# BioinformaticsToolsmith/MeShClust

Measured on AMD Instinct MI355X. Metric: sequences clustered/sec (+ NW cell-updates/sec) at 1/2/4/8 MI355X, higher is better.
Workload: dtype u8

## Files before the change

include/meshclust_amd.h:

```cpp
#ifndef MESHCLUST_AMD_H
#define MESHCLUST_AMD_H

#include <stddef.h>
#include <stdint.h>

#ifdef __cplusplus
extern "C" {
#endif

#define MC_ABI_VERSION 1

#define MC_OK 0
#define MC_ERR_ARG 1
#define MC_ERR_HIP 2
#define MC_ERR_STATE 3
#define MC_ERR_OOM 4
#define MC_ERR_INPUT 5
#define MC_ERR_UNSUPPORTED 6
#define MC_ERR_TIMEOUT 7

#define MC_FEAT_ALIGN (1 << 0)
#define MC_FEAT_LD (1 << 1)
#define MC_FEAT_MANHATTAN (1 << 2)
#define MC_FEAT_INTERSECTION (1 << 4)
// ... 46 lines not shown
                   const uint64_t *exc_pos, const uint8_t *exc_val, uint64_t nexc, const int32_t *seg,
                   const uint64_t *seg_off);

int mc_kmer_max(mc_ctx *ctx, int k, uint64_t *largest);

int mc_kmer_build(mc_ctx *ctx, int k, int width_bytes);

int mc_get_histograms(mc_ctx *ctx, void *hist, uint64_t *mags);

int mc_distance_keys(mc_ctx *ctx, const uint32_t *pivots, uint32_t npiv, const uint32_t *ids,
                     uint64_t m, uint16_t *keys);

int mc_split_begin(mc_ctx *ctx, const uint32_t *pivots, uint32_t npiv, const uint32_t *order, uint64_t n);
int mc_split_begin_words(mc_ctx *ctx, const uint64_t *words, uint32_t narr, uint64_t n, int depth);
int mc_split_select(mc_ctx *ctx, uint64_t nq, const uint32_t *arr, const uint64_t *pos, uint32_t *ids);
int mc_split_select_words(mc_ctx *ctx, uint64_t nq, const uint32_t *arr, const uint64_t *pos, uint64_t *words);
int mc_split_end(mc_ctx *ctx);

int mc_pair_features(mc_ctx *ctx, const uint32_t *a, const uint32_t *b, uint64_t m,
                     const uint16_t *flags, int nflag, double *raw);

int mc_set_classifier(mc_ctx *ctx, const mc_classifier *cls);

int mc_classify_pairs(mc_ctx *ctx, const uint32_t *a, const uint32_t *b, uint64_t m,
                      uint8_t *similar, double *combo0, double *sum);

#define MC_ASSIGN_NONE 0xffffffffu
int mc_assign(mc_ctx *ctx, const uint32_t *centre_ids, uint32_t C, const uint32_t *query_ids, uint64_t M,
              double sim, uint32_t *best, double *best_val, uint32_t *n_similar, uint64_t *stats);

int mc_revcomp_rows(mc_ctx *ctx, const uint32_t *ids, uint64_t m, void *rows );

#define MC_STRAND_PLUS 1
#define MC_STRAND_MINUS 2
int mc_assign_strands(mc_ctx *ctx, const uint32_t *centre_ids, uint32_t C, const uint32_t *query_ids, uint64_t M,
                      double sim, int strands , uint32_t *best, double *best_val,
                      uint8_t *strand , uint32_t *n_similar, uint64_t *stats);

int mc_kmer_max_strands(mc_ctx *ctx, int k, int strands , uint64_t *largest);
int mc_kmer_build_strands(mc_ctx *ctx, int k, int width_bytes, int strands );
int mc_orient_pairs(mc_ctx *ctx, const uint32_t *a, const uint32_t *b, uint64_t m, uint8_t *strand ,
                    uint64_t *sad );

#define MC_ASSIGN_MAX_TOP 8
int mc_assign_top(mc_ctx *ctx, const uint32_t *centre_ids, uint32_t C, const uint32_t *query_ids, uint64_t M,
                  double sim, int strands , uint32_t K ,
                  uint32_t *hit , double *hit_val , uint8_t *hit_strand ,
                  uint32_t *n_similar , uint64_t *stats );

int mc_nw_identity(mc_ctx *ctx, const uint32_t *a, const uint32_t *b, uint64_t m, double *ident,
                   int32_t *len, int32_t *ids);

int mc_nw_identity_raw(mc_ctx *ctx, const uint8_t *a, const uint64_t *a_off, const uint8_t *b,
                       const uint64_t *b_off, uint64_t m, double *ident, int32_t *len,
                       int32_t *ids, int32_t *score);

int mc_revcomp_sequences(mc_ctx *ctx, const uint32_t *ids, uint64_t m, uint8_t *bytes, uint64_t *off);

#define MC_IDENT_BATCH_PAIRS (1ull << 20)
#define MC_IDENT_BATCH_BYTES (256ull << 20)
int mc_nw_identity_strands(mc_ctx *ctx, const uint32_t *a, const uint32_t *b, const uint8_t *a_minus, uint64_t m,
                           double *ident, int32_t *len, int32_t *ids);

#define MC_QGRAM_NA 0xffffffffu
int mc_qgram_common(mc_ctx *ctx, const uint32_t *a, const uint32_t *b, const uint8_t *a_minus, uint64_t m, int q,
                    uint32_t *common);

#define MC_CIGAR_I 1u
#define MC_CIGAR_D 2u
#define MC_CIGAR_EQ 7u
#define MC_CIGAR_X 8u
#define MC_ALIGN_BATCH_PAIRS (1ull << 16)
#define MC_ALIGN_SCRATCH_BYTES (1ull << 30)
int mc_nw_align_strands(mc_ctx *ctx, const uint32_t *a, const uint32_t *b, const uint8_t *a_minus, uint64_t m,
                        uint32_t *cigar, uint64_t cap, uint64_t *cig_off ,
                        int32_t *score, int32_t *len, int32_t *ids);
int mc_nw_align_profile(mc_ctx *ctx, double *out , int reset);

int mc_set_align_band(mc_ctx *ctx, int mode );
int mc_nw_band_plan(mc_ctx *ctx, const uint32_t *a, const uint32_t *b, const uint8_t *a_minus, uint64_t m,
                    int32_t *w , int32_t *score );
int mc_nw_band_profile(mc_ctx *ctx, double *out , int reset);

#define MC_PILEUP_CH 8
int mc_nw_pileup_strands(mc_ctx *ctx, const uint32_t *a, const uint32_t *b, const uint8_t *a_minus, uint64_t m,
                         const uint32_t *targets, uint32_t nt, uint64_t *row_off ,
                         uint32_t *table , uint64_t cap_rows,
                         int32_t *score, int32_t *len, int32_t *ids );
int mc_nw_pileup_profile(mc_ctx *ctx, double *out , int reset);

#define MC_QUAL_MAX 93
int mc_load_qualities(mc_ctx *ctx, const uint8_t *qual, uint64_t bytes);
int mc_nw_qpileup_strands(mc_ctx *ctx, const uint32_t *a, const uint32_t *b, const uint8_t *a_minus, uint64_t m,
                          const uint32_t *targets, uint32_t nt, uint64_t *row_off ,
                          uint32_t *table, uint32_t *wtable , uint64_t cap_rows,
                          int32_t *score, int32_t *len, int32_t *ids );

#define MC_MSA_GAP '-'
#define MC_MSA_BATCH_BYTES (256ull << 20)
int mc_nw_msa_begin(mc_ctx *ctx, const uint32_t *a, const uint32_t *b, const uint8_t *a_minus, uint64_t m,
                    const uint32_t *targets, uint32_t nt, uint64_t *row_off ,
                    uint32_t *width , uint64_t *block_width ,
                    int32_t *score, int32_t *len, int32_t *ids );
int mc_nw_msa_rows(mc_ctx *ctx, uint64_t first, uint64_t count, uint8_t *out, uint64_t cap, uint64_t *off );
int mc_nw_msa_end(mc_ctx *ctx);
int mc_nw_msa_profile(mc_ctx *ctx, double *out , int reset);

#define MC_MSA_CH 8
int mc_nw_msa_counts(mc_ctx *ctx, uint32_t first_target, uint32_t ntargets, uint64_t *col_off ,
                     uint32_t *counts, uint32_t *wcounts , uint64_t cap_cols);
int mc_nw_msa_counts_profile(mc_ctx *ctx, double *out , int reset);

int mc_nw_msa_sites(mc_ctx *ctx, const uint64_t *site_off , const uint32_t *sites ,
                    uint64_t first, uint64_t count, uint8_t *alleles, uint8_t *quals , uint64_t cap,
                    uint64_t *off );
int mc_nw_msa_sites_profile(mc_ctx *ctx, double *out , int reset);

#define MC_CROSS_RES 8
#define MC_CROSS_MAX_READ (1u << 18)
#define MC_CROSS_BATCH_CANDS (1ull << 20)
int mc_nw_msa_crossover(mc_ctx *ctx, const uint64_t *x, const uint64_t *y, uint64_t nc, int32_t *out );
int mc_nw_msa_crossover_profile(mc_ctx *ctx, double *out , int reset);

int mc_set_order(mc_ctx *ctx, const uint32_t *order, uint64_t n);
int mc_kill(mc_ctx *ctx, uint64_t pos);
int mc_cluster_begin(mc_ctx *ctx, uint32_t first_id);
int mc_scan(mc_ctx *ctx, uint32_t centre_id, uint64_t S, uint64_t E, uint32_t *flagged_pos,
            uint64_t cap, mc_scan_result *res);

#define MC_SHARD_BLOCK 256
int mc_scan_part(mc_ctx *ctx, uint32_t centre_id, uint64_t S, uint64_t E, uint32_t part, uint32_t nparts,
                 uint32_t *flagged_pos, uint64_t cap, mc_scan_result *res);
int mc_scan_commit(mc_ctx *ctx, const uint32_t *flagged_pos, uint64_t n, mc_scan_result *res);

int mc_align_part(mc_ctx *ctx, uint32_t centre_id, uint64_t S, uint64_t E, uint32_t part, uint32_t nparts,
                  double *ident, uint64_t cap, uint64_t *n_part, uint64_t *pairs, uint64_t *cells);
int mc_scan_ident(mc_ctx *ctx, uint32_t centre_id, uint64_t S, uint64_t E, const double *ident,
                  uint32_t *flagged_pos, uint64_t cap, mc_scan_result *res);

int mc_accumulate(mc_ctx *ctx, const uint32_t *bin_lo, const uint64_t *bounds, uint32_t nbins, double sim,
                  uint32_t *centre_ids, uint64_t *member_off, uint32_t *member_ids, uint64_t *nclusters,
                  uint64_t *stats);

uint64_t mc_mailbox_bytes(int world, uint64_t n);
int mc_set_mailbox(mc_ctx *ctx, void *host, uint64_t bytes, int rank, int world, int share);
int mc_ctx_pci_bus_id(mc_ctx *ctx, char *buf, int len);
int mc_accum_plan_info(mc_ctx *ctx, uint32_t nbins, uint32_t info[4]);
int mc_set_accum_grid(mc_ctx *ctx, uint32_t grid);
int mc_accum_reserve(mc_ctx *ctx, uint32_t nbins);
int mc_ctx_partition(mc_ctx *ctx, int slot, int share);

int mc_mean_shift(mc_ctx *ctx, const uint32_t *centre_ids, uint32_t C, const uint64_t *member_off,
                  const uint32_t *members, int delta, uint32_t *new_centre);

int mc_update_iteration(mc_ctx *ctx, const uint32_t *centre_ids, uint32_t C, const uint64_t *member_off,
                        const uint32_t *members, int delta, uint32_t *new_centre, uint8_t *similar,
                        double *combo0, uint64_t *npairs);

int mc_mean_shift_range(mc_ctx *ctx, const uint32_t *centre_ids, uint32_t C, const uint64_t *member_off,
                        const uint32_t *members, int delta, uint32_t j0, uint32_t j1, uint32_t *new_centre);


int mc_classify_values(mc_ctx *ctx, const double *raw, uint64_t m, uint8_t *similar, double *combo0,
                       double *sum);

int mc_mean_shift_select(mc_ctx *ctx, const uint32_t *centre_ids, uint32_t C, const uint64_t *member_off,
// ... 19 lines not shown
```

meshclust_amd/__init__.py:

```python
import ctypes as C
import os
import subprocess

import numpy as np

HERE = os.path.dirname(os.path.abspath(__file__))
ROOT = os.path.dirname(HERE)
LIB_DIR = os.path.join(HERE, "lib")
BIN = os.path.join(HERE, "bin", "meshclust")
GPU_LIB = os.environ.get("MC_GPU_LIB", os.path.join(LIB_DIR, "libmcgpu.so"))
HOST_LIB = os.path.join(LIB_DIR, "libmeshclust.so")
HEADER = os.path.join(ROOT, "include", "meshclust_amd.h")

FEAT_ALIGN, FEAT_LD, FEAT_MANHATTAN = 1, 2, 4
FEAT_INTERSECTION, FEAT_PEARSON, FEAT_KULCZYNSKI2 = 16, 32, 1024
COMBO_SQUARED, COMBO_SELF = 1, 2
ASSIGN_NONE = 0xFFFFFFFF
MC_STRAND_PLUS, MC_STRAND_MINUS = 1, 2
ASSIGN_MAX_TOP = 8
ERR_ARG, ERR_UNSUPPORTED = 1, 6
ERR_STATE = 3
CIGAR_I, CIGAR_D, CIGAR_EQ, CIGAR_X = 1, 2, 7, 8
PILEUP_CH = 8
MSA_GAP = ord("-")
MSA_CH = 8
CROSS_RES = 8
QUAL_MAX = 93
QGRAM_NA = 0xFFFFFFFF
FAMILIES = ("kmer", "keys", "pairs", "scan", "finalize", "mean_shift", "nw", "layout")


class MCError(RuntimeError):
    pass


def build(jobs=8):
    subprocess.run(["make", "-s", "-j%d" % jobs, "-C", os.path.join(HERE, "csrc")], check=True)


class Classifier(C.Structure):
    _fields_ = [
        ("n_single", C.c_int32),
        ("lookup", C.c_uint16 * 8),
        ("is_sim", C.c_int32 * 8),
        ("mins", C.c_double * 8),
        ("maxs", C.c_double * 8),
        ("n_combo", C.c_int32),
        ("combo_kind", C.c_int32 * 8),
        ("combo_len", C.c_int32 * 8),
        ("combo_idx", (C.c_int32 * 4) * 8),
        ("weights", C.c_double * 9),
    ]


class ScanResult(C.Structure):
    _fields_ = [
        ("is_min", C.c_int32),
        ("has_best", C.c_int32),
        ("best_pos", C.c_uint64),
        ("best_val", C.c_double),
        ("n_flagged", C.c_uint64),
        ("new_centre", C.c_uint32),
        ("n_members", C.c_uint32),
        ("nw_pairs", C.c_uint64),
        ("nw_cells", C.c_uint64),
    ]


_gpu = None
_host = None


def _p(a):
    return a.ctypes.data_as(C.c_void_p) if a is not None else None


def gpu_lib():
    global _gpu
    if _gpu is None:
        if not os.path.exists(GPU_LIB):
            raise ImportError("libmcgpu.so not built (run meshclust_amd.build()); no CPU fallback exists")
        lib = C.CDLL(GPU_LIB)
        lib.mc_last_error.restype = C.c_char_p
        lib.mc_ctx_create.argtypes = [C.c_int, C.POINTER(C.c_void_p)]
        lib.mc_ctx_destroy.argtypes = [C.c_void_p]
        for name in ("mc_load_sequences", "mc_load_packed", "mc_kmer_max", "mc_kmer_build", "mc_get_histograms", "mc_distance_keys",
                     "mc_pair_features", "mc_set_classifier", "mc_classify_pairs", "mc_nw_identity",
                     "mc_nw_identity_raw", "mc_set_order", "mc_kill", "mc_cluster_begin", "mc_scan",
                     "mc_mean_shift", "mc_update_iteration", "mc_timers", "mc_classify_values", "mc_mean_shift_select", "mc_accumulate",
                     "mc_scan_part", "mc_scan_commit", "mc_comm_unique_id", "mc_comm_create", "mc_comm_allgather",
                     "mc_comm_stats", "mc_comm_destroy", "mc_sync", "mc_assign", "mc_assign_strands",
                     "mc_revcomp_rows", "mc_assign_top", "mc_revcomp_sequences", "mc_nw_identity_strands",
                     "mc_nw_align_strands", "mc_nw_align_profile", "mc_nw_pileup_strands", "mc_nw_pileup_profile",
                     "mc_kmer_max_strands", "mc_kmer_build_strands", "mc_orient_pairs", "mc_qgram_common"):
            getattr(lib, name).restype = C.c_int
        lib.mc_comm_create.argtypes = [C.c_int, C.c_int, C.c_int, C.c_char_p, C.POINTER(C.c_void_p)]
        lib.mc_comm_allgather.argtypes = [C.c_void_p, C.c_void_p, C.c_uint64, C.c_void_p]
        lib.mc_comm_stats.argtypes = [C.c_void_p, C.POINTER(C.c_uint64), C.POINTER(C.c_uint64)]
        lib.mc_comm_destroy.argtypes = [C.c_void_p, C.c_int]
        lib.mc_assign.argtypes = [C.c_void_p, C.c_void_p, C.c_uint32, C.c_void_p, C.c_uint64, C.c_double,
                                  C.c_void_p, C.c_void_p, C.c_void_p, C.c_void_p]
        lib.mc_assign_strands.argtypes = [C.c_void_p, C.c_void_p, C.c_uint32, C.c_void_p, C.c_uint64, C.c_double, C.c_int,
                                          C.c_void_p, C.c_void_p, C.c_void_p, C.c_void_p, C.c_void_p]
        lib.mc_revcomp_rows.argtypes = [C.c_void_p, C.c_void_p, C.c_uint64, C.c_void_p]
        lib.mc_assign_top.argtypes = [C.c_void_p, C.c_void_p, C.c_uint32, C.c_void_p, C.c_uint64, C.c_double, C.c_int,
                                      C.c_uint32, C.c_void_p, C.c_void_p, C.c_void_p, C.c_void_p, C.c_void_p]
        lib.mc_revcomp_sequences.argtypes = [C.c_void_p, C.c_void_p, C.c_uint64, C.c_void_p, C.c_void_p]
        lib.mc_nw_identity_strands.argtypes = [C.c_void_p, C.c_void_p, C.c_void_p, C.c_void_p, C.c_uint64, C.c_void_p,
                                               C.c_void_p, C.c_void_p]
        lib.mc_qgram_common.argtypes = [C.c_void_p, C.c_void_p, C.c_void_p, C.c_void_p, C.c_uint64, C.c_int, C.c_void_p]
        lib.mc_nw_align_strands.argtypes = [C.c_void_p, C.c_void_p, C.c_void_p, C.c_void_p, C.c_uint64, C.c_void_p,
                                            C.c_uint64, C.c_void_p, C.c_void_p, C.c_void_p, C.c_void_p]
        lib.mc_nw_align_profile.argtypes = [C.c_void_p, C.c_void_p, C.c_int]
        lib.mc_nw_pileup_strands.argtypes = [C.c_void_p, C.c_void_p, C.c_void_p, C.c_void_p, C.c_uint64, C.c_void_p, C.c_uint32,
                                             C.c_void_p, C.c_void_p, C.c_uint64, C.c_void_p, C.c_void_p, C.c_void_p]
        lib.mc_nw_pileup_profile.argtypes = [C.c_void_p, C.c_void_p, C.c_int]
        lib.mc_kmer_max_strands.argtypes = [C.c_void_p, C.c_int, C.c_int, C.POINTER(C.c_uint64)]
        lib.mc_kmer_build_strands.argtypes = [C.c_void_p, C.c_int, C.c_int, C.c_int]
        lib.mc_orient_pairs.argtypes = [C.c_void_p, C.c_void_p, C.c_void_p, C.c_uint64, C.c_void_p, C.c_void_p]
        lib.mc_load_qualities.restype = C.c_int
        lib.mc_load_qualities.argtypes = [C.c_void_p, C.c_void_p, C.c_uint64]
        lib.mc_nw_qpileup_strands.restype = C.c_int
        lib.mc_nw_qpileup_strands.argtypes = [C.c_void_p, C.c_void_p, C.c_void_p, C.c_void_p, C.c_uint64, C.c_void_p, C.c_uint32,
                                              C.c_void_p, C.c_void_p, C.c_void_p, C.c_uint64, C.c_void_p, C.c_void_p, C.c_void_p]
        for name in ("mc_nw_msa_begin", "mc_nw_msa_rows", "mc_nw_msa_end", "mc_nw_msa_profile"):
            getattr(lib, name).restype = C.c_int
        lib.mc_nw_msa_begin.argtypes = [C.c_void_p, C.c_void_p, C.c_void_p, C.c_void_p, C.c_uint64, C.c_void_p, C.c_uint32,
                                        C.c_void_p, C.c_void_p, C.c_void_p, C.c_void_p, C.c_void_p, C.c_void_p]
        lib.mc_nw_msa_rows.argtypes = [C.c_void_p, C.c_uint64, C.c_uint64, C.c_void_p, C.c_uint64, C.c_void_p]
        lib.mc_nw_msa_end.argtypes = [C.c_void_p]
        lib.mc_nw_msa_profile.argtypes = [C.c_void_p, C.c_void_p, C.c_int]
        lib.mc_nw_msa_counts.restype = C.c_int
        lib.mc_nw_msa_counts.argtypes = [C.c_void_p, C.c_uint32, C.c_uint32, C.c_void_p, C.c_void_p, C.c_void_p, C.c_uint64]
        lib.mc_nw_msa_counts_profile.restype = C.c_int
        lib.mc_nw_msa_counts_profile.argtypes = [C.c_void_p, C.c_void_p, C.c_int]
        lib.mc_nw_msa_sites.restype = C.c_int
        lib.mc_nw_msa_sites.argtypes = [C.c_void_p, C.c_void_p, C.c_void_p, C.c_uint64, C.c_uint64, C.c_void_p, C.c_void_p, C.c_uint64,
                                        C.c_void_p]
        lib.mc_nw_msa_sites_profile.restype = C.c_int
        lib.mc_nw_msa_sites_profile.argtypes = [C.c_void_p, C.c_void_p, C.c_int]
        lib.mc_nw_msa_crossover.restype = C.c_int
        lib.mc_nw_msa_crossover.argtypes = [C.c_void_p, C.c_void_p, C.c_void_p, C.c_uint64, C.c_void_p]
        lib.mc_nw_msa_crossover_profile.restype = C.c_int
        lib.mc_nw_msa_crossover_profile.argtypes = [C.c_void_p, C.c_void_p, C.c_int]
        for name in ("mc_set_align_band", "mc_nw_band_plan", "mc_nw_band_profile"):
            getattr(lib, name).restype = C.c_int
        lib.mc_set_align_band.argtypes = [C.c_void_p, C.c_int]
        lib.mc_nw_band_plan.argtypes = [C.c_void_p, C.c_void_p, C.c_void_p, C.c_void_p, C.c_uint64, C.c_void_p, C.c_void_p]
        lib.mc_nw_band_profile.argtypes = [C.c_void_p, C.c_void_p, C.c_int]
        _bind_steps(lib)
        _gpu = lib
    return _gpu


def _bind_steps(lib):
    vp, u32, u64 = C.c_void_p, C.c_uint32, C.c_uint64
    lib.mc_set_order.argtypes = [vp, vp, u64]
    lib.mc_kill.argtypes = [vp, u64]
    lib.mc_cluster_begin.argtypes = [vp, u32]
    lib.mc_scan.argtypes = [vp, u32, u64, u64, vp, u64, C.POINTER(ScanResult)]
    lib.mc_scan_part.argtypes = [vp, u32, u64, u64, u32, u32, vp, u64, C.POINTER(ScanResult)]
    lib.mc_scan_commit.argtypes = [vp, vp, u64, C.POINTER(ScanResult)]
    lib.mc_align_part.argtypes = [vp, u32, u64, u64, u32, u32, vp, u64, C.POINTER(u64), C.POINTER(u64), C.POINTER(u64)]
    lib.mc_scan_ident.argtypes = [vp, u32, u64, u64, vp, vp, u64, C.POINTER(ScanResult)]
    lib.mc_mean_shift_range.argtypes = [vp, vp, u32, vp, vp, C.c_int, u32, u32, vp]
    for name in ("mc_set_order", "mc_kill", "mc_cluster_begin", "mc_scan", "mc_scan_part", "mc_scan_commit",
                 "mc_align_part", "mc_scan_ident", "mc_mean_shift_range", "mc_mean_shift"):
        getattr(lib, name).restype = C.c_int
    lib.mc_last_error.restype = C.c_char_p


def load_engine_lib(path):
    lib = C.CDLL(path)
    lib.mc_ctx_create.argtypes = [C.c_int, C.POINTER(C.c_void_p)]
    lib.mc_ctx_destroy.argtypes = [C.c_void_p]
    _bind_steps(lib)
    return lib


def host_lib():
    global _host
    if _host is None:
        if not os.path.exists(HOST_LIB):
            raise ImportError("libmeshclust.so not built (run meshclust_amd.build())")
        gpu_lib()
        lib = C.CDLL(HOST_LIB)
        lib.mcl_parse.restype = C.c_void_p
        lib.mcl_parse.argtypes = [C.POINTER(C.c_char_p), C.c_int, C.c_int, C.c_char_p, C.c_int]
        lib.mcl_parse_q.restype = C.c_void_p
        lib.mcl_parse_q.argtypes = lib.mcl_parse.argtypes
        lib.mcl_qualities.restype = None
        lib.mcl_qualities.argtypes = [C.c_void_p, C.POINTER(C.c_void_p), C.POINTER(C.c_uint64)]
        lib.mcl_num_seqs.restype = C.c_uint64
# ... 299 lines not shown
        r = ScanResult()
        rc = self.lib.mc_scan_part(self.ctx, int(centre), int(S), int(E), int(part), int(nparts), _p(fl), cap, C.byref(r))
        return rc, _scan_dict(r), fl[:min(int(r.n_flagged), cap)].copy() if rc == 0 else fl[:0]

    def scan_commit(self, flagged):
        fl = np.ascontiguousarray(flagged, np.uint32)
        r = ScanResult()
        rc = self.lib.mc_scan_commit(self.ctx, _p(fl) if len(fl) else None, len(fl), C.byref(r))
        return rc, _scan_dict(r)

    def align_part(self, centre, S, E, part, nparts, cap=None):
        cap = max(int(E) - int(S) + 1, 1) if cap is None else int(cap)
        ident = np.zeros(max(cap, 1))
        n, pairs, cells = C.c_uint64(0), C.c_uint64(0), C.c_uint64(0)
        rc = self.lib.mc_align_part(self.ctx, int(centre), int(S), int(E), int(part), int(nparts), _p(ident), cap,
                                    C.byref(n), C.byref(pairs), C.byref(cells))
        return rc, ident[:min(n.value, cap)].copy() if rc == 0 else ident[:0], pairs.value, cells.value

    def scan_ident(self, centre, S, E, ident, cap=None):
        cap = max(int(E) - int(S) + 1, 1) if cap is None else int(cap)
        ident = np.ascontiguousarray(ident, np.float64)
        fl = np.zeros(max(cap, 1), np.uint32)
        r = ScanResult()
        rc = self.lib.mc_scan_ident(self.ctx, int(centre), int(S), int(E), _p(ident), _p(fl), cap, C.byref(r))
        return rc, _scan_dict(r), fl[:min(int(r.n_flagged), cap)].copy() if rc == 0 else fl[:0]

    def mean_shift_range(self, centres, member_off, members, delta, j0, j1):
        centres = np.ascontiguousarray(centres, np.uint32)
        member_off = np.ascontiguousarray(member_off, np.uint64)
        members = np.ascontiguousarray(members, np.uint32)
        out = np.zeros(max(int(j1) - int(j0), 1), np.uint32)
        rc = self.lib.mc_mean_shift_range(self.ctx, _p(centres), len(centres), _p(member_off), _p(members), int(delta),
                                          int(j0), int(j1), _p(out))
        return rc, out[:max(int(j1) - int(j0), 0)]

    def mean_shift_select(self, centres, member_off, members, delta, keep):
        centres = np.ascontiguousarray(centres, np.uint32)
        member_off = np.ascontiguousarray(member_off, np.uint64)
        members = np.ascontiguousarray(members, np.uint32)
        keep = np.ascontiguousarray(keep, np.uint8)
        out = np.zeros(len(centres), np.uint32)
        self._ck(self.lib.mc_mean_shift_select(self.ctx, _p(centres), len(centres), _p(member_off), _p(members), delta,
                                             _p(keep), _p(out)), "mc_mean_shift_select")
        return out

    def nw_identity(self, a, b):
        a = np.ascontiguousarray(a, np.uint32)
        b = np.ascontiguousarray(b, np.uint32)
        ident = np.zeros(len(a))
        ln = np.zeros(len(a), np.int32)
        ids = np.zeros(len(a), np.int32)
        self._ck(self.lib.mc_nw_identity(self.ctx, _p(a), _p(b), C.c_uint64(len(a)), _p(ident), _p(ln), _p(ids)),
               "mc_nw_identity")
        return ident, ln, ids

    def revcomp_sequences(self, ids):
        ids = np.ascontiguousarray(ids, np.uint32)
        off = np.zeros(len(ids) + 1, np.uint64)
        self._ck(self.lib.mc_revcomp_sequences(self.ctx, _p(ids), len(ids), None, _p(off)), "mc_revcomp_sequences")
        out = np.zeros(int(off[-1]), np.uint8)
        self._ck(self.lib.mc_revcomp_sequences(self.ctx, _p(ids), len(ids), _p(out), _p(off)), "mc_revcomp_sequences")
        return out, off

    def nw_identity_strands(self, a, b, a_minus=None):
        a = np.ascontiguousarray(a, np.uint32)
        b = np.ascontiguousarray(b, np.uint32)
        am = None if a_minus is None else np.ascontiguousarray(a_minus, np.uint8)
        assert am is None or len(am) == len(a)
        ident = np.zeros(len(a))
        ln = np.zeros(len(a), np.int32)
        ids = np.zeros(len(a), np.int32)
        self._ck(self.lib.mc_nw_identity_strands(self.ctx, _p(a), _p(b), _p(am), C.c_uint64(len(a)), _p(ident), _p(ln),
                                               _p(ids)), "mc_nw_identity_strands")
        return ident, ln, ids

    def qgram_common(self, a, b, q, a_minus=None):
        a = np.ascontiguousarray(a, np.uint32)
        b = np.ascontiguousarray(b, np.uint32)
        am = None if a_minus is None else np.ascontiguousarray(a_minus, np.uint8)
        assert len(a) == len(b) and (am is None or len(am) == len(a))
        out = np.zeros(len(a), np.uint32)
        self._ck(self.lib.mc_qgram_common(self.ctx, _p(a), _p(b), _p(am), C.c_uint64(len(a)), int(q), _p(out)), "mc_qgram_common")
        return out

    def nw_align_strands(self, a, b, a_minus=None, cigar=True):
        a = np.ascontiguousarray(a, np.uint32)
        b = np.ascontiguousarray(b, np.uint32)
        am = None if a_minus is None else np.ascontiguousarray(a_minus, np.uint8)
        assert len(b) == len(a) and (am is None or len(am) == len(a))
        m = len(a)
        off = np.zeros(m + 1, np.uint64)
        sc = np.zeros(m, np.int32)
        ln = np.zeros(m, np.int32)
        ids = np.zeros(m, np.int32)
        if not cigar:
            self._ck(self.lib.mc_nw_align_strands(self.ctx, _p(a), _p(b), _p(am), C.c_uint64(m), None, C.c_uint64(0), _p(off),
                                                _p(sc), _p(ln), _p(ids)), "mc_nw_align_strands")
            return None, off, sc, ln, ids
        cap = 0
        for x in (a, b):
            self._ck(self.lib.mc_revcomp_sequences(self.ctx, _p(x), m, None, _p(off)), "mc_revcomp_sequences")
            cap += int(off[-1])
        words = np.zeros(cap, np.uint32)
        self._ck(self.lib.mc_nw_align_strands(self.ctx, _p(a), _p(b), _p(am), C.c_uint64(m), _p(words), C.c_uint64(cap), _p(off),
                                            _p(sc), _p(ln), _p(ids)), "mc_nw_align_strands")
        return words[:int(off[-1])], off, sc, ln, ids

    def nw_align_profile(self, reset=False):
        out = np.zeros(3)
        self._ck(self.lib.mc_nw_align_profile(self.ctx, _p(out), 1 if reset else 0), "mc_nw_align_profile")
        return float(out[0]), float(out[1]), float(out[2])

    def set_align_band(self, mode):
        self._ck(self.lib.mc_set_align_band(self.ctx, int(mode)), "mc_set_align_band")

    def nw_band_plan(self, a, b, a_minus=None):
        a = np.ascontiguousarray(a, np.uint32)
        b = np.ascontiguousarray(b, np.uint32)
        am = None if a_minus is None else np.ascontiguousarray(a_minus, np.uint8)
        assert len(b) == len(a) and (am is None or len(am) == len(a))
        w = np.zeros(len(a), np.int32)
        sc = np.zeros(len(a), np.int32)
        self._ck(self.lib.mc_nw_band_plan(self.ctx, _p(a), _p(b), _p(am), C.c_uint64(len(a)), _p(w), _p(sc)), "mc_nw_band_plan")
        return w, sc

    def nw_band_profile(self, reset=False):
        out = np.zeros(5)
        self._ck(self.lib.mc_nw_band_profile(self.ctx, _p(out), 1 if reset else 0), "mc_nw_band_profile")
        return int(out[0]), int(out[1]), int(out[2]), float(out[3]), int(out[4])

    def nw_pileup_strands(self, a, b, a_minus, targets, table=True):
        a = np.ascontiguousarray(a, np.uint32)
        b = np.ascontiguousarray(b, np.uint32)
        am = None if a_minus is None else np.ascontiguousarray(a_minus, np.uint8)
        tg = np.ascontiguousarray(targets, np.uint32)
        assert len(b) == len(a) and (am is None or len(am) == len(a))
        m, nt = len(a), len(tg)
        off = np.zeros(nt + 1, np.uint64)
        sc = np.zeros(m, np.int32)
        ln = np.zeros(m, np.int32)
        ids = np.zeros(m, np.int32)
        self._ck(self.lib.mc_nw_pileup_strands(self.ctx, _p(a), _p(b), _p(am), C.c_uint64(m), _p(tg), C.c_uint32(nt), _p(off), None,
                                             C.c_uint64(0), None, None, None), "mc_nw_pileup_strands")
        if not table:
            return None, off, sc, ln, ids
        rows = int(off[-1])
        tab = np.zeros((rows, PILEUP_CH), np.uint32)
        self._ck(self.lib.mc_nw_pileup_strands(self.ctx, _p(a), _p(b), _p(am), C.c_uint64(m), _p(tg), C.c_uint32(nt), _p(off),
                                             _p(tab), C.c_uint64(rows), _p(sc), _p(ln), _p(ids)), "mc_nw_pileup_strands")
        return tab, off, sc, ln, ids

    def load_qualities(self, q):
        q = np.ascontiguousarray(q, np.uint8)
        self._ck(self.lib.mc_load_qualities(self.ctx, _p(q), C.c_uint64(len(q))), "mc_load_qualities")

    def nw_qpileup_strands(self, a, b, a_minus, targets):
        a = np.ascontiguousarray(a, np.uint32)
        b = np.ascontiguousarray(b, np.uint32)
        am = None if a_minus is None else np.ascontiguousarray(a_minus, np.uint8)
        tg = np.ascontiguousarray(targets, np.uint32)
        assert len(b) == len(a) and (am is None or len(am) == len(a))
        m, nt = len(a), len(tg)
        off = np.zeros(nt + 1, np.uint64)
        sc = np.zeros(m, np.int32)
        ln = np.zeros(m, np.int32)
        ids = np.zeros(m, np.int32)
# ... 297 lines not shown
```

meshclust_amd/csrc/gpu/abi.hip:

```cpp
#include <hip/hip_runtime.h>

#include <algorithm>
#include <chrono>
#include <cfloat>
#include <cmath>
#include <cstdio>
#include <cstdlib>
#include <cstring>
#include <map>
#include <mutex>
#include <string>
#include <thread>
#include <vector>

#include "abi_util.hpp"
#include "mcgpu.hpp"

namespace mcg {

static thread_local std::string g_err;

void set_error(const std::string &m) { g_err = m; }

int hip_fail(hipError_t e, const char *what) {
// ... 147 lines not shown
  MCG_CHECK(hipStreamSynchronize(s));
  if (pinned) {
    size_t off = 0;
    for (const DPart &p : parts)
      if (p.h && p.bytes) {
        memcpy(p.h, c->h_dstage + off, p.bytes);
        off += (p.bytes + 255) / 256 * 256;
      }
  }
  return MC_OK;
}

int download_pinned(mc_ctx *c, const void *d, size_t bytes, hipStream_t s, uint8_t **h) {
  *h = nullptr;
  if (bytes > c->h_dstage_cap) {
    if (c->h_dstage) (void)hipHostFree(c->h_dstage);
    c->h_dstage = nullptr;
    c->h_dstage_cap = 0;
    const size_t cap = std::max<size_t>(bytes, 1u << 20);
    if (hipHostMalloc((void **)&c->h_dstage, cap, hipHostMallocDefault) != hipSuccess) {
      (void)hipGetLastError();
      c->h_dstage = nullptr;
      return MC_OK;
    }
    c->h_dstage_cap = cap;
  }
  if (d) {
    MCG_CHECK(hipMemcpyAsync(c->h_dstage, d, bytes, hipMemcpyDeviceToHost, s));
    MCG_CHECK(hipStreamSynchronize(s));
  }
  *h = c->h_dstage;
  return MC_OK;
}

}

using namespace mcg;

extern "C" {

const char *mc_last_error(void) { return mcg::g_err.c_str(); }
int mc_abi_version(void) { return MC_ABI_VERSION; }

int mc_ctx_create(int device, mc_ctx **out) {
  if (!out) return MC_ERR_ARG;
  int ndev = 0;
  hipError_t e = hipGetDeviceCount(&ndev);
  if (e != hipSuccess || ndev == 0) {
    set_error("no HIP device available (libmcgpu requires an MI355X / gfx950 GPU)");
    return MC_ERR_HIP;
  }
  if (device < 0 || device >= ndev) {
    set_error("device index out of range");
    return MC_ERR_ARG;
  }
  MCG_CHECK(hipSetDevice(device));
  hipDeviceProp_t prop;
  MCG_CHECK(hipGetDeviceProperties(&prop, device));
  if (std::string(prop.gcnArchName).find("gfx950") == std::string::npos) {
    set_error(std::string("libmcgpu is built for gfx950, device is ") + prop.gcnArchName);
    return MC_ERR_HIP;
  }
  auto *c = new mc_ctx();
  c->device = device;
  MCG_CHECK(hipStreamCreateWithFlags(&c->stream, hipStreamNonBlocking));
  MCG_CHECK(hipEventCreate(&c->ev0));
  MCG_CHECK(hipEventCreate(&c->ev1));
  c->cls.thr = decision_threshold();
  *out = c;
  return MC_OK;
}

static void mailbox_detach(mc_ctx *c);

int mc_ctx_destroy(mc_ctx *c) {
  if (!c) return MC_OK;
  (void)hipSetDevice(c->device);
  (void)hipStreamSynchronize(c->stream);
  mailbox_detach(c);
  for (Buf *b : {&c->codes, &c->seq_off, &c->seg, &c->seg_off, &c->packed, &c->pk_off, &c->impure, &c->hist, &c->mag, &c->sumsq, &c->len, &c->order,
                 &c->alive, &c->members, &c->member_keys, &c->partials, &c->scan_dev, &c->flags_out, &c->s_a, &c->s_b,
                 &c->s_c, &c->s_d, &c->s_e, &c->s_f, &c->s_g, &c->s_h, &c->s_i, &c->s_j, &c->s_k, &c->hs, &c->mag_s, &c->sumsq_s, &c->len_s, &c->ticket,
                 &c->msum, &c->ident_s, &c->al_a, &c->al_b, &c->al_out, &c->al_id, &c->ord_ids, &c->acc_out, &c->sp_words, &c->sp_keys,
                 &c->sp_scr, &c->sp_nodes, &c->sp_nn, &c->sp_q, &c->sp_err, &c->u_off, &c->u_mem, &c->nw_items, &c->nw_gran, &c->rc_seq, &c->tr_choice, &c->tr_bnd, &c->tr_ops, &c->tr_pairs, &c->tr_res, &c->tr_idx, &c->tr_dst,
                 &c->tr_out, &c->tr_err, &c->bs_pairs, &c->bs_bnd, &c->bs_score, &c->pu_table, &c->pu_diff, &c->pu_rows, &c->pu_toff, &c->pu_roff, &c->qual, &c->pu_wtable, &c->pu_qoff, &c->msa_width, &c->msa_col, &c->msa_words, &c->msa_bw, &c->msa_rec, &c->msa_out, &c->msa_cnt, &c->msa_wcnt, &c->msa_cdiff, &c->msa_crec, &c->msa_ctgt, &c->msa_scol, &c->msa_sres, &c->msa_stgt, &c->msa_srec, &c->msa_sout, &c->msa_sq, &c->msa_xrec, &c->msa_xout, &c->hist_fwd, &c->or_runs})
    release(*b);
  if (c->h_scan) (void)hipHostFree(c->h_scan);
  if (c->h_stage) (void)hipHostFree(c->h_stage);
  if (c->h_dstage) (void)hipHostFree(c->h_dstage);
  if (c->h_res) (void)hipHostFree(c->h_res);
  for (auto e : c->ev_pool) (void)hipEventDestroy(e);
  (void)hipEventDestroy(c->ev0);
  (void)hipEventDestroy(c->ev1);
  (void)hipStreamDestroy(c->stream);
  delete c;
  return MC_OK;
}

static int load_common(mc_ctx *c, const uint64_t *seq_off, uint64_t n, const int32_t *seg, const uint64_t *seg_off,
                       std::vector<uint64_t> &pk_off) {
  MCG_CHECK(hipSetDevice(c->device));
  for (uint64_t i = 0; i < n; i++)
    if (seq_off[i + 1] < seq_off[i] || seg_off[i + 1] < seg_off[i]) {
      set_error("offsets must be non-decreasing");
      return MC_ERR_ARG;
    }
  c->n = n;
  c->k = 0;
  c->kmer_spec_k = 0;
  c->canon = false;
  release(c->hist_fwd);
  c->h_seq_off.assign(seq_off, seq_off + n + 1);
  if (pk_off.empty()) {
    pk_off.resize(n + 1);
    pk_off[0] = 0;
    for (uint64_t i = 0; i < n; i++) pk_off[i + 1] = pk_off[i] + (seq_off[i + 1] - seq_off[i] + 15) / 16;
  }
  TRY(ensure(c->codes, seq_off[n] + 16));
  TRY(ensure(c->packed, pk_off[n] * 4 + 16));
  TRY(ensure(c->impure, n + 16));
  TRY(upload(c, c->pk_off, pk_off.data(), n + 1, c->stream));
  TRY(upload(c, c->seq_off, seq_off, n + 1, c->stream));
  TRY(upload(c, c->seg, seg, 2 * seg_off[n], c->stream));
  TRY(upload(c, c->seg_off, seg_off, n + 1, c->stream));
  return MC_OK;
}

int mc_load_sequences(mc_ctx *c, const uint8_t *codes, const uint64_t *seq_off, uint64_t n, const int32_t *seg,
                      const uint64_t *seg_off) {
  if (c) {
    c->h_uoff.clear();
    c->h_umem.clear();
    c->has_qual = false;
    msa_drop(c);
  }
  if (!c || !seq_off || !seg_off || (n && !codes)) return MC_ERR_ARG;
  std::vector<uint64_t> pk_off;
  TRY(load_common(c, seq_off, n, seg, seg_off, pk_off));
  if (seq_off[n]) MCG_CHECK(hipMemcpyAsync(c->codes.p, codes, seq_off[n], hipMemcpyHostToDevice, c->stream));
  if (n) TRY(launch_pack(c));
  MCG_CHECK(hipStreamSynchronize(c->stream));
  flush_timers(c);
  return MC_OK;
}

int mc_load_packed(mc_ctx *c, const uint32_t *packed, const uint64_t *pk_off, const uint64_t *seq_off, uint64_t n,
                   const uint64_t *exc_pos, const uint8_t *exc_val, uint64_t nexc, const int32_t *seg,
                   const uint64_t *seg_off) {
  if (c) {
    c->h_uoff.clear();
    c->h_umem.clear();
    c->has_qual = false;
    msa_drop(c);
  }
  if (!c || !pk_off || !seq_off || !seg_off || (n && !packed) || (nexc && (!exc_pos || !exc_val))) return MC_ERR_ARG;
  for (uint64_t i = 0; i < n; i++)
    if (pk_off[i + 1] - pk_off[i] != (seq_off[i + 1] - seq_off[i] + 15) / 16) {
      set_error("pk_off must give every record ceil(length / 16) words");
      return MC_ERR_ARG;
    }
  std::vector<uint8_t> imp(n, 0);
  for (uint64_t q = 0, i = 0; q < nexc; q++) {
    if (exc_pos[q] >= seq_off[n] || (q && exc_pos[q] <= exc_pos[q - 1])) {
      set_error("exception positions must be ascending and inside the sequences");
      return MC_ERR_ARG;
    }
    while (seq_off[i + 1] <= exc_pos[q]) i++;
    imp[i] = 1;
  }
  std::vector<uint64_t> pko(pk_off, pk_off + n + 1);
  TRY(load_common(c, seq_off, n, seg, seg_off, pko));
  if (pk_off[n]) MCG_CHECK(hipMemcpyAsync(c->packed.p, packed, pk_off[n] * 4, hipMemcpyHostToDevice, c->stream));
  if (n) MCG_CHECK(hipMemcpyAsync(c->impure.p, imp.data(), n, hipMemcpyHostToDevice, c->stream));
  if (nexc) {
    TRY(ensure(c->s_a, nexc * 8 + 16));
    TRY(ensure(c->s_b, nexc + 16));
// ... 806 lines not shown
  mailbox_detach(c);
  if (world == 0) return MC_OK;
  if (!host || world < 1 || world > 64 || rank < 0 || rank >= world || share < 1 || share > world ||
      ((uintptr_t)host & 7))
    return MC_ERR_ARG;
  {
    std::lock_guard<std::mutex> lk(g_mb_mu);
    auto it = g_mb_refs.find(host);
    if (it == g_mb_refs.end()) {
      const hipError_t e = hipHostRegister(host, bytes, hipHostRegisterMapped | hipHostRegisterPortable);
      if (e != hipSuccess) return hip_fail(e, "hipHostRegister (mailbox)");
      g_mb_refs[host] = 1;
    } else {
      it->second++;
    }
  }
  void *dev = nullptr;
  const hipError_t e = hipHostGetDevicePointer(&dev, host, 0);
  if (e != hipSuccess) {
    c->mb_host = host;
    mailbox_detach(c);
    return hip_fail(e, "hipHostGetDevicePointer (mailbox)");
  }
  c->mb_host = host;
  c->mb_dev = dev;
  c->mb_bytes = bytes;
  c->mb_rank = rank;
  c->mb_world = world;
  c->mb_share = share;
  return MC_OK;
}

int mc_accum_plan_info(mc_ctx *c, uint32_t nbins, uint32_t info[4]) {
  if (!c || !info || nbins == 0) return MC_ERR_ARG;
  if (!c->has_cls || c->norder == 0) return MC_ERR_STATE;
  if (!fused(c) || !accum_plan_info(c, nbins, info)) {
    set_error("device-resident accumulation does not take this configuration");
    return MC_ERR_UNSUPPORTED;
  }
  return MC_OK;
}

int mc_set_accum_grid(mc_ctx *c, uint32_t grid) {
  if (!c) return MC_ERR_ARG;
  c->acc_grid = grid;
  return MC_OK;
}

int mc_accum_reserve(mc_ctx *c, uint32_t nbins) {
  if (!c || nbins == 0) return MC_ERR_ARG;
  if (!c->has_cls || c->norder == 0) return MC_ERR_STATE;
  if (!fused(c)) {
    set_error("device-resident accumulation does not take this configuration");
    return MC_ERR_UNSUPPORTED;
  }
  MCG_CHECK(hipSetDevice(c->device));
  return accum_reserve(c, nbins);
}

int mc_ctx_partition(mc_ctx *c, int slot, int share) {
  if (!c || share < 1 || share > 32 || slot < 0 || slot >= share) return MC_ERR_ARG;
  if (slot == c->part_slot && share == c->part_share) return MC_OK;
  MCG_CHECK(hipSetDevice(c->device));
  MCG_CHECK(hipStreamSynchronize(c->stream));
  int cus = 0;
  MCG_CHECK(hipDeviceGetAttribute(&cus, hipDeviceAttributeMultiprocessorCount, c->device));
  hipStream_t s = nullptr;
  int n = 0;
  if (share == 1) {
    MCG_CHECK(hipStreamCreateWithFlags(&s, hipStreamNonBlocking));
  } else {
    std::vector<uint32_t> mask((size_t)(cus + 31) / 32, 0u);
    for (int i = 0; i < cus; i++)
      if ((i / 8) % share == slot) {
        mask[(size_t)i / 32] |= 1u << (i % 32);
        n++;
      }
    if (n < 16) {
      set_error("mc_ctx_partition: fewer than 16 CUs per slot");
      return MC_ERR_ARG;
    }
    MCG_CHECK(hipExtStreamCreateWithCUMask(&s, (uint32_t)mask.size(), mask.data()));
  }
  (void)hipStreamDestroy(c->stream);
  c->stream = s;
  c->part_slot = slot;
  c->part_share = share;
  c->part_cus = share == 1 ? 0 : n;
  return MC_OK;
}

int mc_accumulate(mc_ctx *c, const uint32_t *bin_lo, const uint64_t *bounds, uint32_t nbins, double sim,
                  uint32_t *centre_ids, uint64_t *member_off, uint32_t *member_ids, uint64_t *nclusters,
                  uint64_t *stats) {
  if (!c || !c->has_cls || c->norder == 0) return MC_ERR_STATE;
  if (!bin_lo || !bounds || nbins == 0 || bin_lo[nbins] != c->norder || !centre_ids || !member_off || !member_ids ||
      !nclusters)
    return MC_ERR_ARG;
  for (uint32_t b = 0; b < nbins; b++)
    if (bin_lo[b] > bin_lo[b + 1]) return MC_ERR_ARG;
  if (!fused(c) || !accum_supported(c, nbins)) {
    set_error("device-resident accumulation does not take this configuration");
    return MC_ERR_UNSUPPORTED;
  }
  if (c->mb_world > 0 && c->mb_bytes < mc_mailbox_bytes(c->mb_world, c->norder)) {
    set_error("mailbox smaller than mc_mailbox_bytes(world, n)");
    return MC_ERR_ARG;
  }
  MCG_CHECK(hipSetDevice(c->device));
  const uint64_t n = c->norder;
  TRY(upload(c, c->s_d, bin_lo, (size_t)nbins + 1, c->stream));
  TRY(upload(c, c->s_e, bounds, nbins, c->stream));
  TRY(ensure(c->s_f, n * 4 + 16));
  TRY(ensure(c->s_g, (n + 1) * 8 + 16));
  TRY(ensure(c->acc_out, 256));
  MCG_CHECK(hipMemsetAsync(c->acc_out.p, 0, 256, c->stream));
  TRY(launch_accum(c, (const uint32_t *)c->s_d.p, (const uint64_t *)c->s_e.p, nbins, sim, (uint32_t *)c->members.p,
                   (uint64_t *)c->member_keys.p, (uint32_t *)c->s_f.p, (uint64_t *)c->s_g.p,
                   (uint64_t *)c->acc_out.p));
  uint64_t out[32];
  TRY(download_parts(c, {{out, c->acc_out.p, 256}}, c->stream));
  flush_timers(c);
  if (out[3]) {
    set_error(out[3] == 99 ? "device accumulation: hand-off timed out"
              : out[3] == 11 ? "bvec_iterator dereference out of range (the reference throws here)"
                             : "tried incrementing null iterator (the reference throws here)");
    return out[3] == 99 ? MC_ERR_TIMEOUT : MC_ERR_INPUT;
  }
  const uint64_t ncl = out[0], nmem = out[4];
  if (ncl > n || nmem != n) {
    set_error("device accumulation produced an inconsistent partition");
    return MC_ERR_HIP;
  }
  TRY(ensure(c->ord_ids, n * 4 + 16));
  TRY(launch_order_members(c, (const uint64_t *)c->member_keys.p, (const uint32_t *)c->members.p,
                           (const uint64_t *)c->s_g.p, ncl, (uint32_t *)c->ord_ids.p));
  TRY(download_parts(c, {{member_ids, c->ord_ids.p, n * 4}, {centre_ids, c->s_f.p, ncl * 4},
                         {member_off, c->s_g.p, (ncl + 1) * 8}}, c->stream));
  const uint64_t om = order_members_max();
  for (uint64_t k = 0; k < ncl; k++) {
    const uint64_t a = member_off[k], b = member_off[k + 1];
    if (b - a <= om) continue;
    std::vector<uint64_t> kk(b - a);
    std::vector<uint32_t> pp(b - a);
    TRY(download_parts(c, {{kk.data(), (const uint64_t *)c->member_keys.p + a, (b - a) * 8},
                           {pp.data(), (const uint32_t *)c->members.p + a, (b - a) * 4}}, c->stream));
    for (uint64_t i = 0; i < b - a; i++)
      if (kk[i] == 0) kk[i] = pp[i];
    std::sort(kk.begin(), kk.end());
    for (uint64_t i = a; i < b; i++) member_ids[i] = c->h_order[(uint32_t)kk[i - a]];
  }
  for (uint64_t k = 0; k < ncl; k++) centre_ids[k] = c->h_order[centre_ids[k]];
  *nclusters = ncl;
  if (stats) {
    stats[0] = out[1];
    stats[1] = out[2];
    for (int i = 0; i < 3; i++) stats[2 + i] = out[5 + i] / 100;
  }
  if (getenv("MC_ACCUM_PROFILE")) {
    fprintf(stderr, "[accum] steps %llu window %.3f (centre data %.3f window %.3f record %.3f) wait %.3f collect %.3f "
            "(stragglers+reduce %.3f column sums %.3f [takes %.3f] mean %.3f closest %.3f) ms\n",
            (unsigned long long)out[1], out[5] / 1e5, out[12] / 1e5, out[13] / 1e5, out[14] / 1e5, out[6] / 1e5,
            out[7] / 1e5, out[8] / 1e5, out[9] / 1e5, out[15] / 1e5, out[10] / 1e5, out[11] / 1e5);
    fprintf(stderr, "[accum] closest: members scored %.3f, reduced %.3f, winner %.3f ms\n", out[18] / 1e5, out[19] / 1e5,
            out[20] / 1e5);
    fprintf(stderr, "[accum] window: record span %.3f, record stores issued %.3f ms\n", out[21] / 1e5, out[22] / 1e5);
// ... 245 lines not shown
```

meshclust_amd/csrc/gpu/abi_align.hip:

```cpp
#include <hip/hip_runtime.h>

#include <cstdlib>
#include <cstring>
#include <string>
#include <vector>

#include "../host/band.hpp"
#include "../host/pairbatch.hpp"
#include "abi_util.hpp"
#include "mcgpu.hpp"

using namespace mcg;

namespace {

mc::PairBatchCaps batch_caps(const char *pairs_env, uint64_t pairs, bool scratch) {
  return {pairs_env ? env_cap(pairs_env, pairs) : pairs, env_cap("MC_IDENT_BYTES", MC_IDENT_BATCH_BYTES),
          scratch ? env_cap("MC_ALIGN_SCRATCH", MC_ALIGN_SCRATCH_BYTES) : 0};
}

int revseq_batch(mc_ctx *c, const uint32_t *ids, uint32_t u, std::vector<uint64_t> &h_off) {
  h_off.resize((size_t)u + 1);
  h_off[0] = 0;
  for (uint32_t r = 0; r < u; r++)
    h_off[r + 1] = h_off[r] + (c->h_seq_off[ids[r] + 1] - c->h_seq_off[ids[r]] + 15) / 16 * 16;
  TRY(ensure(c->rc_seq, h_off[u] + 16));
  TRY(upload(c, c->s_h, ids, u, c->stream));
  TRY(upload(c, c->s_i, h_off.data(), (size_t)u + 1, c->stream));
  return launch_revseq(c, (const uint32_t *)c->s_h.p, u, (const uint64_t *)c->s_i.p, h_off[u], (uint8_t *)c->rc_seq.p);
}

void scatter_res(const std::vector<int32_t> &res, uint64_t i0, uint64_t mb, int32_t *score, int32_t *len, int32_t *ids) {
  for (uint64_t k = 0; k < mb; k++) {
    if (score) score[i0 + k] = res[k * TRACE_RES];
    if (len) len[i0 + k] = res[k * TRACE_RES + 1];
    if (ids) ids[i0 + k] = res[k * TRACE_RES + 2];
  }
}

constexpr uint64_t BAND_W0 = 64, BAND_BND_BYTES = 256ull << 20;

uint64_t band_w0() {
  const char *e = getenv("MC_BAND_W0");
  const long long v = e ? atoll(e) : 0;
  return v >= 1 ? (uint64_t)std::min<long long>(v, 1 << 27) : BAND_W0;
}

int band_search(mc_ctx *c, const uint32_t *a, const uint32_t *b, const uint8_t *a_minus, uint64_t m, int32_t *w, int32_t *score) {
  const uint64_t w0 = band_w0();
  mc::PairBatcher pb(c->h_seq_off.data(), c->n, a, b, a_minus, m, batch_caps("MC_IDENT_BATCH", MC_IDENT_BATCH_PAIRS, false));
  std::vector<uint64_t> h_off, wcur;
  std::vector<TracePair> recs;
  std::vector<uint64_t> todo, next;
  std::vector<int32_t> sc;
  auto planned = [&](uint64_t i, int64_t la, int64_t lb, int32_t S) {
    score[i] = S;
    w[i] = mc::band_plan(la, lb, S);
    c->band_stat[w[i] >= 0 ? 0 : 1] += 1;
    if (w[i] >= 0) c->band_stat[3] += w[i];
  };
  while (pb.next()) {
    if (!pb.uniq.empty()) TRY(revseq_batch(c, pb.uniq.data(), (uint32_t)pb.uniq.size(), h_off));
    todo.clear();
    wcur.assign(pb.i1 - pb.i0, w0);
    for (uint64_t i = pb.i0; i < pb.i1; i++) {
      const int64_t la = (int64_t)pb.length(a[i]), lb = (int64_t)pb.length(b[i]);
      if (la == 0)
        planned(i, la, lb, lb > 0 ? (int32_t)mc::band_neg_inf(la, lb) : 0);
      else if (lb == 0)
        planned(i, la, lb, (int32_t)(-2 - la));
      else
        todo.push_back(i);
    }
    while (!todo.empty()) {
      sc.resize(todo.size());
      for (size_t at = 0, end; at < todo.size(); at = end) {
        recs.clear();
        uint64_t bnd = 0;
        for (end = at; end < todo.size(); end++) {
          const uint64_t i = todo[end], la = pb.length(a[i]), lb = pb.length(b[i]);
          const uint64_t need = mc::band_bnd_ints(la, lb, wcur[i - pb.i0]);
          if (end > at && (bnd + need) * 4 > BAND_BND_BYTES) break;
          TracePair pr{};
          pr.a_off = pb.minus(i) ? h_off[pb.slot(a[i])] : c->h_seq_off[a[i]];
          pr.b_off = c->h_seq_off[b[i]];
          pr.bnd_off = bnd;
          pr.la = (uint32_t)la;
          pr.lb = (uint32_t)lb;
          pr.a_rc = pb.minus(i) ? 1 : 0;
          pr.r = mc::BAND_R;
// ... 797 lines not shown
int mc_revcomp_sequences(mc_ctx *c, const uint32_t *ids, uint64_t m, uint8_t *bytes, uint64_t *off) {
  if (!c || !c->codes.p) return MC_ERR_STATE;
  if (!off || (m && !ids)) return MC_ERR_ARG;
  TRY(check_ids(c, ids, m));
  off[0] = 0;
  for (uint64_t i = 0; i < m; i++) off[i + 1] = off[i] + (c->h_seq_off[ids[i] + 1] - c->h_seq_off[ids[i]]);
  if (!bytes || m == 0) return MC_OK;
  MCG_CHECK(hipSetDevice(c->device));
  const std::vector<uint8_t> all_minus(m, 1);
  mc::PairBatcher pb(c->h_seq_off.data(), c->n, ids, nullptr, all_minus.data(), m, batch_caps(nullptr, MC_IDENT_BATCH_PAIRS, false));
  std::vector<uint64_t> h_off;
  std::vector<uint8_t> host;
  while (pb.next()) {
    const uint32_t u = (uint32_t)pb.uniq.size();
    TRY(revseq_batch(c, pb.uniq.data(), u, h_off));
    host.resize(h_off[u]);
    if (h_off[u]) MCG_CHECK(hipMemcpyAsync(host.data(), c->rc_seq.p, h_off[u], hipMemcpyDeviceToHost, c->stream));
    MCG_CHECK(hipStreamSynchronize(c->stream));
    for (uint64_t i = pb.i0; i < pb.i1; i++)
      if (off[i + 1] > off[i]) memcpy(bytes + off[i], host.data() + h_off[pb.slot(ids[i])], off[i + 1] - off[i]);
  }
  flush_timers(c);
  return MC_OK;
}

int mc_nw_identity_strands(mc_ctx *c, const uint32_t *a, const uint32_t *b, const uint8_t *a_minus, uint64_t m,
                           double *ident, int32_t *len, int32_t *ids) {
  if (!c || !c->codes.p) return MC_ERR_STATE;
  if (m == 0) return MC_OK;
  MCG_CHECK(hipSetDevice(c->device));
  TRY(check_ids(c, a, m));
  TRY(check_ids(c, b, m));
  mc::PairBatcher pb(c->h_seq_off.data(), c->n, a, b, a_minus, m, batch_caps("MC_IDENT_BATCH", MC_IDENT_BATCH_PAIRS, false));
  std::vector<uint32_t> ai, bi, out;
  std::vector<uint64_t> h_off, a_off2, la[2], lb[2];
  while (pb.next()) {
    const uint64_t i0 = pb.i0, mb = pb.i1 - pb.i0, nm = pb.nminus, np = mb - nm;
    ai.resize(mb);
    bi.resize(mb);
    out.resize(mb);
    for (int s = 0; s < 2; s++) {
      la[s].clear();
      lb[s].clear();
    }
    uint64_t km = 0, kp = nm;
    for (uint64_t i = i0; i < pb.i1; i++) {
      const bool minus = pb.minus(i);
      const uint64_t k = minus ? km++ : kp++;
      ai[k] = minus ? 2 * pb.slot(a[i]) : a[i];
      bi[k] = b[i];
      out[k] = (uint32_t)(i - i0);
      la[minus].push_back(pb.length(a[i]));
      lb[minus].push_back(pb.length(b[i]));
    }
    if (nm) {
      TRY(revseq_batch(c, pb.uniq.data(), (uint32_t)pb.uniq.size(), h_off));
      a_off2.resize(2 * pb.uniq.size());
      for (size_t r = 0; r < pb.uniq.size(); r++) {
        a_off2[2 * r] = h_off[r];
        a_off2[2 * r + 1] = h_off[r] + pb.length(pb.uniq[r]);
      }
      TRY(upload(c, c->s_j, a_off2.data(), a_off2.size(), c->stream));
    }
    TRY(upload(c, c->s_d, ai.data(), mb, c->stream));
    TRY(upload(c, c->s_e, bi.data(), mb, c->stream));
    TRY(upload(c, c->s_g, out.data(), mb, c->stream));
    TRY(ensure(c->s_f, mb * 16 + 64));
    double *d_id = (double *)c->s_f.p;
    int32_t *d_len = (int32_t *)(d_id + mb), *d_ids = d_len + mb;
    const uint32_t *d_ai = (const uint32_t *)c->s_d.p, *d_bi = (const uint32_t *)c->s_e.p, *d_out = (const uint32_t *)c->s_g.p;
    if (nm)
      TRY(launch_nw(c, (uint8_t *)c->rc_seq.p, (uint64_t *)c->s_j.p, d_ai, (uint8_t *)c->codes.p, (uint64_t *)c->seq_off.p, d_bi,
                    nm, la[1], lb[1], d_id, d_len, d_ids, nullptr, d_out));
    if (np)
      TRY(launch_nw(c, (uint8_t *)c->codes.p, (uint64_t *)c->seq_off.p, d_ai + nm, (uint8_t *)c->codes.p,
                    (uint64_t *)c->seq_off.p, d_bi + nm, np, la[0], lb[0], d_id, d_len, d_ids, nullptr, d_out + nm));
    TRY(download_parts(c, {{ident ? ident + i0 : nullptr, d_id, mb * 8}, {len ? len + i0 : nullptr, d_len, mb * 4},
                           {ids ? ids + i0 : nullptr, d_ids, mb * 4}}, c->stream));
  }
  flush_timers(c);
  return MC_OK;
}

int mc_nw_align_strands(mc_ctx *c, const uint32_t *a, const uint32_t *b, const uint8_t *a_minus, uint64_t m,
                        uint32_t *cigar, uint64_t cap, uint64_t *cig_off, int32_t *score, int32_t *len, int32_t *ids) {
  if (!c || !c->codes.p) return MC_ERR_STATE;
  if (!cig_off) return MC_ERR_ARG;
  if (m == 0) {
    cig_off[0] = 0;
    return MC_OK;
  }
  if (!a || !b) return MC_ERR_ARG;
  MCG_CHECK(hipSetDevice(c->device));
  TRY(check_ids(c, a, m));
  TRY(check_ids(c, b, m));
  std::vector<int32_t> plan;
  TRY(align_plan(c, a, b, a_minus, m, plan));
  TRY(align_check_caps(c, "mc_nw_align_strands", a, b, m, plan));
  std::vector<uint32_t> words, nops(m);
  std::vector<uint64_t> dst;
  TRY(align_batches(c, "mc_nw_align_strands", a, b, a_minus, m, plan, [&](uint64_t i0, uint64_t mb, const std::vector<int32_t> &res) {
    scatter_res(res, i0, mb, score, len, ids);
    dst.resize(mb);
    uint64_t tot = 0;
    for (uint64_t k = 0; k < mb; k++) {
      dst[k] = tot;
      nops[i0 + k] = (uint32_t)res[k * TRACE_RES + 3];
      tot += nops[i0 + k];
    }
    if (cigar && tot) {
      TRY(ensure(c->tr_out, tot * 4 + 64));
      TRY(upload(c, c->tr_dst, dst.data(), mb, c->stream));
      TRY(launch_nw_pack(c, (uint32_t)mb, (const TracePair *)c->tr_pairs.p, (const uint32_t *)c->tr_ops.p,
                         (const int32_t *)c->tr_res.p, (const uint64_t *)c->tr_dst.p, (uint32_t *)c->tr_out.p));
      const size_t at = words.size();
      words.resize(at + tot);
      MCG_CHECK(hipMemcpyAsync(words.data() + at, c->tr_out.p, tot * 4, hipMemcpyDeviceToHost, c->stream));
      MCG_CHECK(hipStreamSynchronize(c->stream));
    }
    return (int)MC_OK;
  }));
  flush_timers(c);
  cig_off[0] = 0;
  for (uint64_t i = 0; i < m; i++) cig_off[i + 1] = cig_off[i] + nops[i];
  if (cigar) {
    if (cap < cig_off[m]) {
      set_error("mc_nw_align_strands: cigar holds " + std::to_string(cap) + " words, the alignments have " +
                std::to_string(cig_off[m]));
      return MC_ERR_ARG;
    }
    if (!words.empty()) memcpy(cigar, words.data(), words.size() * 4);
  }
  return MC_OK;
}

int mc_nw_pileup_strands(mc_ctx *c, const uint32_t *a, const uint32_t *b, const uint8_t *a_minus, uint64_t m,
                         const uint32_t *targets, uint32_t nt, uint64_t *row_off, uint32_t *table, uint64_t cap_rows,
                         int32_t *score, int32_t *len, int32_t *ids) {
  return pileup_call(c, "mc_nw_pileup_strands", false, a, b, a_minus, m, targets, nt, row_off, table, nullptr, cap_rows, score, len,
                     ids);
}

int mc_nw_qpileup_strands(mc_ctx *c, const uint32_t *a, const uint32_t *b, const uint8_t *a_minus, uint64_t m,
                          const uint32_t *targets, uint32_t nt, uint64_t *row_off, uint32_t *table, uint32_t *wtable,
                          uint64_t cap_rows, int32_t *score, int32_t *len, int32_t *ids) {
  return pileup_call(c, "mc_nw_qpileup_strands", true, a, b, a_minus, m, targets, nt, row_off, table, wtable, cap_rows, score, len,
                     ids);
}

int mc_load_qualities(mc_ctx *c, const uint8_t *qual, uint64_t bytes) {
  if (!c || !c->codes.p) return MC_ERR_STATE;
  const uint64_t want = c->h_seq_off.empty() ? 0 : c->h_seq_off.back();
  if (bytes != want || (bytes && !qual)) {
    set_error("mc_load_qualities: " + std::to_string(bytes) + " values, the loaded sequences have " + std::to_string(want) + " bytes");
    return MC_ERR_ARG;
  }
  for (uint64_t i = 0; i < bytes; i++)
    if (qual[i] > MC_QUAL_MAX) {
      set_error("mc_load_qualities: value " + std::to_string((int)qual[i]) + " at byte " + std::to_string(i) + " is above MC_QUAL_MAX");
      return MC_ERR_ARG;
    }
  MCG_CHECK(hipSetDevice(c->device));
  TRY(ensure(c->qual, bytes + 64));
  if (bytes) MCG_CHECK(hipMemcpyAsync(c->qual.p, qual, bytes, hipMemcpyHostToDevice, c->stream));
  MCG_CHECK(hipStreamSynchronize(c->stream));
  c->has_qual = true;
// ... 72 lines not shown
```

meshclust_amd/csrc/gpu/mcgpu.hpp:

```cpp
#pragma once
#include <hip/hip_runtime.h>

#include <cstdint>
#include <string>
#include <vector>

#include "../../../include/meshclust_amd.h"

namespace mcg {

__device__ __forceinline__ int wave_id() { return __builtin_amdgcn_readfirstlane((int)(threadIdx.x >> 6)); }

enum Family { F_KMER = 0, F_KEYS, F_PAIRS, F_SCAN, F_FINAL, F_MSHIFT, F_NW, F_LAYOUT, F_NFAM, F_NW_FWD = F_NFAM, F_NW_TB, F_NW_PU, F_NW_MSAW, F_NW_MSAR, F_NW_MSAC, F_NW_BAND, F_NW_MSAS, F_NW_CROSS, F_NALL };

struct DevClassifier {
  mc_classifier c;
  double thr;
  int align;
  int layout;
};

struct FastCls {
  double rinv[MC_MAX_SINGLE], noff[MC_MAX_SINGLE], nsgn[MC_MAX_SINGLE], range[MC_MAX_SINGLE];
  double rB;
// ... 62 lines not shown
struct MsaCountTarget {
  uint64_t c_off, row0, col0, drow0;
  uint32_t L, W, depth, pad;
};

struct MsaSiteTarget {
  uint64_t row0, s_off;
  uint32_t L, S;
};

struct MsaSitePair {
  uint64_t a_off, w_off, row0, s_off, out_off, q_off;
  uint32_t la, lb, nw, S, a_rc, pad;
};

struct CrossPair {
  uint64_t xw_off, yw_off;
  uint32_t la, xnw, ynw, minus, out, pad;
};

struct SplitNode {
  int64_t lo, hi, cut;
  int32_t depth, left, fin, pad;
};

struct HostScan {
  mc_scan_result r;
  uint32_t seq;
  uint32_t pad;
  uint32_t flags[1];
};

}

struct mc_ctx {
  int device = 0;
  hipStream_t stream = nullptr;
  uint8_t *h_stage = nullptr;
  uint8_t *h_dstage = nullptr;
  size_t h_dstage_cap = 0;
  size_t stage_off = 0;
  uint64_t n = 0;
  std::vector<uint64_t> h_seq_off;
  mcg::Buf codes, seq_off, seg, seg_off;
  mcg::Buf packed, pk_off, impure;
  int kmer_spec_k = 0;
  int k = 0, B = 0, width = 0;
  uint64_t pitch = 0;
  mcg::Buf hist, mag, sumsq, len;
  bool canon = false;
  mcg::Buf hist_fwd, or_runs;
  mcg::DevClassifier cls{};
  mcg::FastCls fcls{};
  bool has_cls = false;
  uint64_t norder = 0;
  mcg::Buf order, alive, members, member_keys, partials, scan_dev, flags_out;
  uint32_t step = 0;
  mcg::ScanDev *h_scan = nullptr;
  size_t h_scan_cap = 0;
  mcg::Buf hs, mag_s, sumsq_s, len_s, ticket, msum;
  uint64_t npad = 0;
  mcg::HostScan *h_res = nullptr, *h_res_dev = nullptr;
  size_t h_res_cap = 0;
  uint32_t seq = 0;
  std::vector<uint64_t> pending_kills;
  bool pending_begin = false;
  uint64_t pending_first_pos = 0;
  std::vector<uint64_t> h_spos;
  std::vector<uint32_t> h_order;
  std::vector<uint8_t> h_alive;
  mcg::Buf ident_s, al_a, al_b, al_out, al_id, ord_ids;
  mcg::Buf acc_out;
  mcg::Buf sp_words, sp_keys, sp_scr, sp_nodes, sp_nn, sp_q, sp_err;
  uint64_t sp_n = 0;
  uint32_t sp_narr = 0;
  int sp_depth0 = 0;
  void *mb_host = nullptr, *mb_dev = nullptr;
  uint64_t mb_bytes = 0;
  int mb_rank = 0, mb_world = 0, mb_share = 1;
  uint32_t acc_grid = 0;
  int part_slot = 0, part_share = 1, part_cus = 0;
  mcg::Buf s_a, s_b, s_c, s_d, s_e, s_f, s_g, s_h, s_i, s_j, s_k;
  mcg::Buf nw_items, nw_gran;
  mcg::Buf rc_seq;
  mcg::Buf tr_choice, tr_bnd, tr_ops, tr_pairs, tr_res, tr_idx, tr_dst, tr_out, tr_err;
  double tr_choice_bytes = 0;
  int align_band = 0;
  mcg::Buf bs_pairs, bs_bnd, bs_score;
  double band_stat[4] = {0, 0, 0, 0};
  mcg::Buf pu_table, pu_diff, pu_rows, pu_toff, pu_roff;
  mcg::Buf qual, pu_wtable, pu_qoff;
  bool has_qual = false;
  bool msa_on = false;
  mcg::Buf msa_width, msa_col, msa_words, msa_bw, msa_rec, msa_out, msa_cnt, msa_wcnt, msa_cdiff, msa_crec, msa_ctgt;
  mcg::Buf msa_scol, msa_sres, msa_stgt, msa_srec, msa_sout, msa_sq, msa_xrec, msa_xout;
  std::vector<uint32_t> msa_a, msa_b, msa_targets, msa_tof, msa_nops, msa_tp;
  std::vector<uint64_t> msa_tp_off;
  std::vector<uint8_t> msa_minus;
  std::vector<uint64_t> msa_woff, msa_row_off, msa_W;
  mcg::Buf u_off, u_mem;
  std::vector<uint64_t> h_uoff;
  std::vector<uint32_t> h_umem;
  std::vector<void *> pinned;
  hipEvent_t ev0 = nullptr, ev1 = nullptr;
  std::vector<hipEvent_t> ev_pool;
  std::vector<std::pair<int, int>> ev_pending;
  int ev_open = -1;
  double fam_ms[mcg::F_NALL] = {0};
  double fam_n[mcg::F_NALL] = {0};
};

namespace mcg {

void set_error(const std::string &m);
int hip_fail(hipError_t e, const char *what);
int ensure(Buf &b, size_t bytes);
void timed_begin(mc_ctx *c);
void timed_end(mc_ctx *c, Family f);
void flush_timers(mc_ctx *c);

HistView hist_view(const mc_ctx *c);

int launch_expand(mc_ctx *c, uint64_t nexc, const uint64_t *d_exc_pos, const uint8_t *d_exc_val);
int launch_pack(mc_ctx *c);
int launch_kmer(mc_ctx *c, int k, int width, bool write, uint64_t *d_max, int *d_err);
int launch_distance_keys(mc_ctx *c, const uint32_t *d_piv, uint32_t npiv, const uint32_t *d_ids, uint64_t m,
                         uint16_t *d_keys);
constexpr int32_t SPLIT_MAXNODE = 32768;
int split_build_words(mc_ctx *c, const uint32_t *d_order, uint64_t n, uint32_t npiv, const uint16_t *d_keys,
                      uint64_t *d_words);
int launch_order_members(mc_ctx *c, const uint64_t *d_keys, const uint32_t *d_pos, const uint64_t *d_cl_off, uint64_t ncl,
                         uint32_t *d_ids);
uint64_t order_members_max();
int stage_h2d(mc_ctx *c, void *dst, const void *src, size_t bytes);
int launch_select(mc_ctx *c, uint64_t *d_words, uint64_t n, uint32_t *d_scr, SplitNode *d_nodes, int32_t *d_nnodes,
                  int32_t maxnode, int32_t depth0, uint32_t ngroups, const uint32_t *d_qarr, const uint64_t *d_qoff,
                  const uint64_t *d_qpos, uint64_t *d_qout, int *d_err);
int launch_pairs(mc_ctx *c, const uint32_t *d_a, const uint32_t *d_b, uint64_t m, const uint16_t *flags, int nflag,
                 double *d_raw, uint8_t *d_sim, double *d_c0, double *d_sum, bool classify);
int launch_scan(mc_ctx *c, uint32_t centre, uint64_t S, uint64_t E, const double *d_ident, int *nblocks);
int launch_merge_pairs(mc_ctx *c, const uint32_t *d_new, uint32_t C, const uint64_t *d_poff, uint32_t *d_a,
                       uint32_t *d_b);
int launch_values(mc_ctx *c, const double *d_raw, uint64_t m, uint8_t *d_sim, double *d_c0, double *d_sum);
int launch_finalize(mc_ctx *c, int nblocks);
int launch_mean_shift(mc_ctx *c, const uint32_t *d_cid, uint32_t C, const uint64_t *d_off, const uint64_t *h_off,
                      const uint32_t *d_mem, int delta, const uint8_t *d_keep, uint32_t *d_new, uint32_t j0,
                      uint32_t j1);
int build_static(mc_ctx *c);
bool accum_supported(const mc_ctx *c, uint32_t nb);
bool accum_plan_info(const mc_ctx *c, uint32_t nb, uint32_t info[4]);
uint64_t mailbox_slot_granules(uint32_t world, uint64_t n);
const void *accum_fn_dense(int width, int nch, bool prof);
const void *accum_fn_dstream(int width, int nch, bool prof);
const void *accum_fn_wide(int width, bool prof);
const void *accum_fn_chunk(int width, int nch, bool compact);
int accum_reserve(mc_ctx *c, uint32_t nb);
int launch_accum(mc_ctx *c, const uint32_t *d_bin_lo, const uint64_t *d_bounds, uint32_t nb, double sim,
                 uint32_t *d_mem_pos, uint64_t *d_mkeys, uint32_t *d_cl_centre, uint64_t *d_cl_off, uint64_t *d_out);
int launch_fused_scan(mc_ctx *c, uint32_t centre, uint64_t S, uint64_t E, uint32_t seq, const double *d_ident,
                      uint32_t part = 0, uint32_t nparts = 0);
int launch_commit(mc_ctx *c, const uint32_t *d_flags, uint32_t nflag, uint32_t seq);
int launch_nw(mc_ctx *c, const uint8_t *d_A, const uint64_t *d_aoff, const uint32_t *d_ai, const uint8_t *d_B,
              const uint64_t *d_boff, const uint32_t *d_bi, uint64_t m, const std::vector<uint64_t> &h_alen,
              const std::vector<uint64_t> &h_blen, double *d_ident, int32_t *d_len, int32_t *d_ids,
              int32_t *d_score, const uint32_t *d_out = nullptr);
int launch_revseq(mc_ctx *c, const uint32_t *d_ids, uint32_t u, const uint64_t *d_out_off, uint64_t out_bytes,
                  uint8_t *d_out);

int launch_canon_rows(mc_ctx *c, const uint8_t *d_in, uint8_t *d_out, uint64_t *d_max);
int launch_orient(mc_ctx *c, const uint8_t *d_fwd, const uint32_t *d_a, const uint32_t *h_b, uint64_t m, Buf &runs,
                  uint8_t *d_strand, uint64_t *d_sad);

int nw_trace_rows(uint64_t la);
uint64_t nw_trace_choice_bytes(uint64_t la, uint64_t lb);
int launch_nw_trace(mc_ctx *c, const std::vector<TracePair> &h_pairs, const TracePair *d_pairs, const uint8_t *d_rc,
                    uint8_t *d_choice, int *d_bnd, uint32_t *d_ops, int32_t *d_res, int *d_err);
int launch_nw_pack(mc_ctx *c, uint32_t m, const TracePair *d_pairs, const uint32_t *d_ops, const int32_t *d_res,
                   const uint64_t *d_dst, uint32_t *d_out);

int launch_nwband_forward(mc_ctx *c, const TraceArgs &q);
int launch_nwband_traceback(mc_ctx *c, const TraceArgs &q);
int launch_nwband_scores(mc_ctx *c, uint32_t m, const TracePair *d_pairs, const uint8_t *d_rc, int *d_bnd, int32_t *d_score);

int launch_nw_pileup(mc_ctx *c, uint32_t m, const TracePair *d_pairs, const uint8_t *d_rc, const uint32_t *d_ops,
                     const int32_t *d_res, const uint64_t *d_rowbase, uint32_t *d_table, int32_t *d_deq, int32_t *d_ddel,
                     bool naive);
int launch_nw_pileup_finish(mc_ctx *c, uint32_t nt, const uint64_t *d_tgt_off, const uint64_t *d_row_off, uint32_t *d_table,
                            const int32_t *d_deq, const int32_t *d_ddel);
int launch_nw_qpileup(mc_ctx *c, uint32_t m, const TracePair *d_pairs, const uint8_t *d_rc, const uint32_t *d_ops,
                      const int32_t *d_res, const uint64_t *d_rowbase, const uint64_t *d_qoff, uint32_t *d_table,
                      uint32_t *d_wtable, int32_t *d_deq, int32_t *d_ddel);

int launch_msa_width(mc_ctx *c, uint32_t m, const TracePair *d_pairs, const uint32_t *d_ops, const int32_t *d_res,
                     const uint64_t *d_rowbase, uint32_t *d_width);
int launch_msa_columns(mc_ctx *c, uint32_t nt, const uint64_t *d_row_off, const uint32_t *d_width, uint32_t *d_col, uint64_t *d_bw);
int launch_msa_render(mc_ctx *c, uint64_t nrows, const MsaRow *d_rows, const uint8_t *d_rc, const uint32_t *d_words,
                      const uint32_t *d_width, const uint32_t *d_col, uint8_t *d_out);
int launch_msa_counts(mc_ctx *c, uint64_t npairs, const MsaCountPair *d_pairs, const uint8_t *d_rc, const uint32_t *d_words,
                      const uint32_t *d_width, const uint32_t *d_col, uint32_t *d_counts, uint32_t *d_wcounts, int32_t *d_deq,
                      int32_t *d_ddel);
int launch_msa_counts_finish(mc_ctx *c, uint32_t nt, const MsaCountTarget *d_tgts, const uint32_t *d_width, const uint32_t *d_col,
                             uint32_t *d_counts, const int32_t *d_deq, const int32_t *d_ddel);
int launch_msa_sites_resolve(mc_ctx *c, uint32_t nt, const MsaSiteTarget *d_tgts, const uint32_t *d_width, const uint32_t *d_col,
                             const uint32_t *d_sites, uint2 *d_res);
int launch_msa_sites(mc_ctx *c, uint64_t npairs, const MsaSitePair *d_pairs, const uint8_t *d_rc, const uint32_t *d_words,
                     const uint32_t *d_width, const uint32_t *d_col, const uint32_t *d_sites, const uint2 *d_res, uint8_t *d_out,
                     uint8_t *d_qout);
int launch_crossover(mc_ctx *c, uint32_t nc, const CrossPair *d_cands, const uint32_t *d_words, uint32_t max_la, int32_t *d_out);
void msa_drop(mc_ctx *c);

}

#define MCG_CHECK(expr)                                   \
  do {                                                    \
    hipError_t _e = (expr);                               \
    if (_e != hipSuccess) return mcg::hip_fail(_e, #expr); \
  } while (0)
```

meshclust_amd/csrc/host/cluster.hpp:

```cpp
#pragma once
#include <cstddef>
#include <cstdint>
#include <string>
#include <vector>

#include "bvec.hpp"
#include "common.hpp"
#include "fasta.hpp"

namespace mc {

struct Center {
  uint32_t centre;
  std::vector<uint32_t> points;
  bool del = false;
};


void fault_point(const ShardComm *comm, const char *stage);

struct ClusterConfig {
  const ShardComm *comm = nullptr;
  double sim = 0.90;
  int iterations = 15;
  int delta = 5;
  bool verbose = true;
  bool align = false;
  int width = 1;
};

struct ClusterStats {
  uint64_t scan_steps = 0;
  uint64_t scan_candidates = 0;
  uint64_t update_evals = 0;
  uint64_t merge_evals = 0;
  uint64_t update_iters_fixed = 0;
  uint64_t update_evals_run = 0;
  uint64_t nw_pairs = 0, nw_cells = 0;
  uint64_t nw_screened = 0;
  uint64_t align_nw_pairs = 0, align_nw_cells = 0;
  std::string accum_path;
  std::string update_path;
};

std::vector<Center> mean_shift_cluster(const Dataset &ds, mc_ctx *ctx, BVec &bv, const ClusterConfig &cfg,
                                       PhaseTimer &timer, ClusterStats &stats);

void write_clstr(const std::string &path, const Dataset &ds, const std::vector<Center> &part, int threads = 1);

}
```

meshclust_amd/csrc/host/common.hpp:

```cpp
#pragma once
#include <chrono>
#include <cstdint>
#include <cstdio>
#include <cstdlib>
#include <map>
#include <stdexcept>
#include <string>
#include <vector>

#include "../../../include/meshclust_amd.h"

extern "C" {
int mc_kmer_max_strands(mc_ctx *, int, int, uint64_t *) __attribute__((weak));
int mc_kmer_build_strands(mc_ctx *, int, int, int) __attribute__((weak));
int mc_orient_pairs(mc_ctx *, const uint32_t *, const uint32_t *, uint64_t, uint8_t *, uint64_t *) __attribute__((weak));
int mc_nw_identity_strands(mc_ctx *, const uint32_t *, const uint32_t *, const uint8_t *, uint64_t, double *, int32_t *,
                           int32_t *) __attribute__((weak));
int mc_qgram_common(mc_ctx *, const uint32_t *, const uint32_t *, const uint8_t *, uint64_t, int, uint32_t *) __attribute__((weak));
}

namespace mc {

struct Error : std::runtime_error {
  int code;
  explicit Error(const std::string &m, int c = 1) : std::runtime_error(m), code(c) {}
};
struct ShardComm {
  int rank = 0, world = 1;
  int (*allgather)(void *user, const void *in, uint64_t bytes, void *out) = nullptr;
  void *user = nullptr;
};

struct PeerError : Error {
  explicit PeerError(const std::string &m) : Error(m, 1) {}
};

void comm_phase(const ShardComm *comm, const char *phase);

inline void check(int rc, const char *what) {
  if (rc != MC_OK) {
    const char *e = mc_last_error();
    throw Error(std::string(what) + " failed: " + (e ? e : "?"), 3);
  }
}

inline void strands_engine_check() {
  if (!mc_kmer_max_strands || !mc_kmer_build_strands || !mc_orient_pairs || !mc_nw_identity_strands)
    throw Error("--both-strands: the engine this program is linked against has no strand-blind histograms "
                "(mc_kmer_max_strands, mc_kmer_build_strands, mc_orient_pairs, mc_nw_identity_strands); "
                "they exist in the GPU engine libmcgpu only",
                1);
}

struct PhaseTimer {
  std::map<std::string, double> ms;
  std::vector<std::string> order;
  void add(const std::string &k, double v) {
    if (!ms.count(k)) order.push_back(k);
    ms[k] += v;
  }
};

inline bool phase_log_on() {
  static const bool on = getenv("MC_PHASE_LOG") && atoi(getenv("MC_PHASE_LOG")) != 0;
  return on;
}

inline double phase_clock_ms() {
  return std::chrono::duration<double, std::milli>(std::chrono::steady_clock::now().time_since_epoch()).count();
}

struct Scope {
  PhaseTimer &t;
  std::string k;
  std::chrono::steady_clock::time_point s;
  Scope(PhaseTimer &tt, std::string kk) : t(tt), k(std::move(kk)), s(std::chrono::steady_clock::now()) {
    if (phase_log_on()) fprintf(stderr, "[phase %p %.3f] + %s\n", (void *)&tt, phase_clock_ms(), k.c_str());
  }
  ~Scope() {
    auto e = std::chrono::steady_clock::now();
    const double v = std::chrono::duration<double, std::milli>(e - s).count();
    t.add(k, v);
    if (phase_log_on()) fprintf(stderr, "[phase %p %.3f] - %s %.3f ms\n", (void *)&t, phase_clock_ms(), k.c_str(), v);
  }
};

}
```

meshclust_amd/csrc/host/runner.cpp:

```cpp
#include "runner.hpp"

#include "model.hpp"

#include <libgen.h>
#include <malloc.h>
#include <sys/stat.h>
#include <unistd.h>

#include <algorithm>
#include <cerrno>
#include <chrono>
#include <cmath>
#include <atomic>
#include <condition_variable>
#include <exception>
#include <mutex>
#include <memory>
#include <thread>
#include <cstdio>
#include <cstdlib>
#include <cstring>
#include <limits>

#ifdef _OPENMP
// ... 259 lines not shown
      const auto b1 = clk::now();
      for (uint32_t id = 0; id < ds.size(); id++) bvp->insert(id);
      const auto b2 = clk::now();
      bvp->insert_finalize(std::max(1, threads / 4));
      const auto b3 = clk::now();
      bvec_ms = std::chrono::duration<double, std::milli>(b3 - b0).count();
      bvec_lap[0] = std::chrono::duration<double, std::milli>(b2 - b1).count();
      bvec_lap[1] = std::chrono::duration<double, std::milli>(b3 - b2).count();
    } catch (...) {
      bvec_err = std::current_exception();
    }
  });
  struct JoinBvec {
    std::thread &t;
    ~JoinBvec() {
      if (t.joinable()) t.join();
    }
  } join_bvec{bvec_thread};
  fault_point(comm, "upload");
  if (upload) {
    Scope s(rr.timer, "upload");
    check(mc_load_packed(ctx, ds.packed.data(), ds.pk_off.data(), ds.seq_off.data(), ds.size(), ds.exc_pos.data(),
                         ds.exc_val.data(), ds.exc_pos.size(), ds.seg.data(), ds.seg_off.data()),
          "mc_load_packed");
  }
  {
    Scope s(rr.timer, "kmer");
    if (opt.both_strands) check(mc_kmer_max_strands(ctx, opt.k, rr.strands, &rr.largest), "mc_kmer_max_strands");
    else check(mc_kmer_max(ctx, opt.k, &rr.largest), "mc_kmer_max");
    int width = rr.largest <= 0xff ? 1 : rr.largest <= 0xffff ? 2 : rr.largest <= 0xffffffffull ? 4 : 8;
    if (const char *fw = getenv("MC_FORCE_WIDTH")) width = std::max(width, atoi(fw));
    rr.width = width;
    if (verbose) printf("Using %d bit histograms\n", 8 * width);
    if (opt.both_strands) check(mc_kmer_build_strands(ctx, opt.k, width, rr.strands), "mc_kmer_build_strands");
    else check(mc_kmer_build(ctx, opt.k, width), "mc_kmer_build");
  }
  comm_phase(comm, "train");
  TrainerConfig tc;
  tc.n_points = opt.sample_size;
  tc.max_pts_from_one = opt.pivots;
  tc.cutoff = opt.similarity;
  tc.k = opt.align ? 0 : opt.k;
  tc.threads = threads;
  tc.verbose = verbose;
  tc.comm = comm;
  tc.both_strands = opt.both_strands;
  {
    Scope s(rr.timer, "len_order.wait");
    if (len_thread.joinable()) len_thread.join();
  }
  if (len_err) std::rethrow_exception(len_err);
  tc.length_order = std::move(len_order);
  Trainer tr(ds, ctx, tc, rr.timer);
  {
    Scope s(rr.timer, "train");
    tr.train();
  }
  {
    Scope s(rr.timer, "bvec.wait");
    bvec_thread.join();
  }
  fault_point(comm, "train");
  rr.timer.add("bvec.overlapped", bvec_ms);
  rr.timer.add("bvec.overlapped.insert", bvec_lap[0]);
  rr.timer.add("bvec.overlapped.finalize", bvec_lap[1]);
  if (bvec_err) std::rethrow_exception(bvec_err);
  mc_classifier cls = tr.classifier();
  check(mc_set_classifier(ctx, &cls), "mc_set_classifier");
  rr.cls = cls;
  rr.similarity = opt.similarity;
  rr.align = opt.align;
  ClusterConfig cc;
  cc.sim = opt.similarity;
  cc.iterations = opt.iterations;
  cc.delta = opt.delta;
  cc.verbose = verbose;
  cc.align = opt.align;
  cc.width = rr.width;
  cc.comm = comm;
  rr.part = mean_shift_cluster(ds, ctx, *bvp, cc, rr.timer, rr.stats);
  rr.stats.nw_pairs = tr.nw_pairs;
  rr.stats.nw_cells = tr.nw_cells;
  rr.stats.nw_screened = tr.nw_screened;
  if (opt.both_strands) {
    Scope s(rr.timer, "orient");
    std::vector<uint32_t> a, b;
    for (const Center &c : rr.part)
      for (uint32_t p : c.points) {
        a.push_back(p);
        b.push_back(c.centre);
      }
    std::vector<uint8_t> st(a.size(), 0);
    std::vector<uint64_t> sad(2 * a.size(), 0);
    check(mc_orient_pairs(ctx, a.data(), b.data(), a.size(), st.data(), sad.data()), "mc_orient_pairs");
    size_t at = 0;
    for (const Center &c : rr.part) {
      rr.member_strand.emplace_back(st.begin() + at, st.begin() + at + c.points.size());
      rr.member_sad.emplace_back(sad.begin() + 2 * at, sad.begin() + 2 * (at + c.points.size()));
      at += c.points.size();
    }
    for (uint8_t v : st) rr.members_minus += v;
  }
  rr.timer.add("total_pipeline",
               std::chrono::duration<double, std::milli>(std::chrono::steady_clock::now() - t0).count());
  return rr;
}

std::string stats_json(const RunResult &rr, double parse_ms, double write_ms) {
  char b[512];
  std::string o;
  snprintf(b, sizeof b, "{\"n\": %zu, \"k\": %d, \"width\": %d, \"clusters\": %zu, \"parse_ms\": %.3f, \"write_ms\": %.3f",
           rr.n, rr.k, rr.width, rr.part.size(), parse_ms, write_ms);
  o += b;
  snprintf(b, sizeof b,
           ", \"scan_steps\": %llu, \"scan_candidates\": %llu, \"update_evals\": %llu, \"merge_evals\": %llu"
           ", \"nw_pairs\": %llu, \"nw_cells\": %llu, \"nw_screened\": %llu, \"align_nw_pairs\": %llu, \"align_nw_cells\": %llu",
           (unsigned long long)rr.stats.scan_steps, (unsigned long long)rr.stats.scan_candidates,
           (unsigned long long)rr.stats.update_evals, (unsigned long long)rr.stats.merge_evals,
           (unsigned long long)rr.stats.nw_pairs, (unsigned long long)rr.stats.nw_cells, (unsigned long long)rr.stats.nw_screened,
           (unsigned long long)rr.stats.align_nw_pairs, (unsigned long long)rr.stats.align_nw_cells);
  o += b;
  if (rr.strands != 1) {
    snprintf(b, sizeof b, ", \"strands\": %d, \"k_auto_length\": %llu, \"members_minus\": %llu", rr.strands,
             (unsigned long long)rr.k_auto_length, (unsigned long long)rr.members_minus);
    o += b;
  }
  o += ", \"accum_path\": \"" + rr.stats.accum_path + "\"";
  if (!rr.stats.update_path.empty()) o += ", \"update_path\": \"" + rr.stats.update_path + "\"";
  o += ", \"update_iters_fixed\": " + std::to_string(rr.stats.update_iters_fixed);
  o += ", \"update_evals_run\": " + std::to_string(rr.stats.update_evals_run);
  o += ", \"phases_ms\": {";
  for (size_t i = 0; i < rr.timer.order.size(); i++) {
    snprintf(b, sizeof b, "%s\"%s\": %.3f", i ? ", " : "", rr.timer.order[i].c_str(), rr.timer.ms.at(rr.timer.order[i]));
    o += b;
  }
  o += "}}";
  return o;
}

void save_model_files(const Options &opt, const Dataset &ds, const RunResult &rr) {
  if (!opt.save_model.empty()) {
    Model m;
    m.k = rr.k;
    m.id = rr.similarity;
    m.align = rr.align ? 1 : 0;
    m.strands = rr.strands;
    m.cls = rr.cls;
    m.centres = rr.part.size();
    write_model(opt.save_model, m);
  }
  if (!opt.save_centres.empty()) {
    std::vector<uint32_t> ids;
    for (const Center &c : rr.part) ids.push_back(c.centre);
    write_fasta(opt.save_centres, ds, ids.data(), ids.size());
  }
}

void write_strands_file(const std::string &path, const Dataset &ds, const RunResult &rr) {
  if (rr.strands == 1 || rr.member_strand.size() != rr.part.size()) throw Error("--strands needs a --both-strands run", 1);
  auto name = [&](uint32_t id) {
    const auto h = ds.headers[id];
    return std::string(h.substr(h.empty() ? 0 : 1));
  };
  std::string out;
  char b[96];
  int label = 0;
  for (size_t c = 0; c < rr.part.size(); c++) {
    const Center &cen = rr.part[c];
    if (cen.points.empty()) continue;
    const std::string cname = name(cen.centre);
    for (size_t j = 0; j < cen.points.size(); j++) {
      snprintf(b, sizeof b, "\t%d\t", label);
      out += name(cen.points[j]) + b + cname;
      snprintf(b, sizeof b, "\t%c\t%llu\t%llu\n", rr.member_strand[c][j] ? '-' : '+',
               (unsigned long long)rr.member_sad[c][2 * j], (unsigned long long)rr.member_sad[c][2 * j + 1]);
      out += b;
    }
    label++;
  }
  FILE *f = fopen(path.c_str(), "w");
  if (!f) throw Error("cannot write " + path + ": " + strerror(errno));
  const bool ok = fwrite(out.data(), 1, out.size(), f) == out.size();
  if (fclose(f) != 0 || !ok) throw Error("cannot write " + path);
}

static void write_stats(const std::string &path, const RunResult &rr, double parse_ms, double write_ms) {
  FILE *f = fopen(path.c_str(), "w");
  if (!f) return;
  fprintf(f, "%s\n", stats_json(rr, parse_ms, write_ms).c_str());
  fclose(f);
}

struct ThreadComm {
  int world;
  std::mutex mu;
  std::condition_variable cv;
  std::vector<uint8_t> buf;
  uint64_t bytes = 0, gen = 0;
  int arrived = 0, left = 0;
  bool draining = false, aborted = false;

  explicit ThreadComm(int w) : world(w) {}
  void abort() {
    std::lock_guard<std::mutex> lk(mu);
    aborted = true;
    cv.notify_all();
  }
  int allgather(int rank, const void *in, uint64_t n, void *out) {
    std::unique_lock<std::mutex> lk(mu);
    cv.wait(lk, [&] { return aborted || !draining; });
    if (aborted) return 1;
    if (arrived == 0) {
      bytes = n;
// ... 136 lines not shown
```

meshclust_amd/csrc/host/trainer.cpp:

```cpp
#include "trainer.hpp"

#include "lazysort.hpp"
#include "qscreen.hpp"

#include <algorithm>
#include <array>
#include <atomic>
#include <cmath>
#include <cstdio>
#include <cstring>
#include <exception>
#include <memory>
#include <set>
#include <thread>

namespace mc {

namespace {

struct ExitZero : Error {
  ExitZero(const std::string &m) : Error(m, 0) {}
};

inline int get_bin(double x, double min_align, double max_align, int num_bins) {
  if (x >= max_align) return num_bins - 1;
  if (x <= min_align) return 0;
  return (int)(num_bins * (x - min_align) / (max_align - min_align));
}

using Labeled = std::pair<PairId, double>;

std::vector<Labeled> resize_vec(const std::vector<Labeled> &vec, size_t new_size, double min_align,
                                double max_align, int num_bins) {
  if (new_size == vec.size()) return vec;
  std::vector<std::vector<Labeled>> bins(num_bins);
  for (const auto &p : vec) bins.at(get_bin(p.second, min_align, max_align, num_bins)).push_back(p);
  std::vector<Labeled> data;
  while (data.size() < new_size) {
    int items_left = (int)(new_size - data.size());
    int take = (int)std::ceil((double)items_left / num_bins);
    for (int i = (int)bins.size() - 1; i >= 0; i--)
      for (int j = 0; j < (int)std::min((size_t)take, bins[i].size()); j++) data.push_back(bins[i][j]);
  }
  return data;
}

std::pair<std::vector<PairId>, std::vector<PairId>> bin_data(const std::vector<Labeled> &vec, double min_align,
                                                             double max_align) {
  const int n_bins = 10;
  std::vector<std::vector<Labeled>> bins(n_bins);
  for (const auto &d : vec) bins.at(get_bin(d.second, min_align, max_align, n_bins)).push_back(d);
  std::vector<PairId> train, test;
  int last = 0;
  for (const auto &bin : bins) {
    for (int i = 0; i < (int)bin.size(); i++) {
      if (i % 2 == last) train.push_back(bin[i].first);
      else test.push_back(bin[i].first);
    }
    last = !last;
  }
  return {train, test};
}

}

bool Trainer::hdr_less(uint32_t a, uint32_t b) const { return ds_.headers[a].compare(ds_.headers[b]) < 0; }

bool Trainer::gather(const std::vector<uint64_t> &mine, std::vector<uint64_t> &all) const {
  const ShardComm *cm = cfg_.comm;
  if (!cm || cm->world <= 1) return false;
  all.assign(mine.size() * (size_t)cm->world, 0);
  if (cm->allgather(cm->user, mine.data(), mine.size() * 8, all.data()) != 0)
    throw PeerError("training all-gather across ranks failed");
  return true;
}

void Trainer::nw_batch(const std::vector<PairId> &pairs, std::vector<double> &ident) {
  std::vector<uint32_t> a(pairs.size()), b(pairs.size());
  for (size_t i = 0; i < pairs.size(); i++) {
    a[i] = pairs[i].first;
    b[i] = pairs[i].second;
  }
  ident.assign(pairs.size(), 0.0);
  if (pairs.empty()) return;
  for (const auto &p : pairs) {
    nw_pairs++;
    nw_cells += ds_.lengths[p.first] * ds_.lengths[p.second];
  }
  if (!cfg_.both_strands) {
    check(mc_nw_identity(ctx_, a.data(), b.data(), pairs.size(), ident.data(), nullptr, nullptr), "mc_nw_identity");
    return;
  }
  strands_engine_check();
  const size_t m = pairs.size();
  for (const auto &p : pairs) {
    nw_pairs++;
    nw_cells += ds_.lengths[p.first] * ds_.lengths[p.second];
  }
  a.insert(a.end(), a.begin(), a.begin() + m);
  b.insert(b.end(), b.begin(), b.begin() + m);
  std::vector<uint8_t> minus(2 * m, 0);
  std::fill(minus.begin() + m, minus.end(), 1);
  std::vector<double> both(2 * m, 0.0);
  check(mc_nw_identity_strands(ctx_, a.data(), b.data(), minus.data(), 2 * m, both.data(), nullptr, nullptr),
        "mc_nw_identity_strands");
  for (size_t i = 0; i < m; i++) ident[i] = both[m + i] > both[i] ? both[m + i] : both[i];
}

void Trainer::screen(const std::vector<PairId> &pairs, int q, bool host, std::vector<char> &out) {
  const size_t m = pairs.size(), S = cfg_.both_strands ? 2 : 1;
  out.assign(m, 0);
  if (m == 0) return;
  std::vector<uint32_t> cnt(S * m, qscreen::NA);
  if (host) {
#pragma omp parallel for schedule(static) num_threads(cfg_.threads)
    for (size_t j = 0; j < S * m; j++) cnt[j] = qscreen::common(ds_, pairs[j % m].first, pairs[j % m].second, j >= m, q);
  } else {
    std::vector<uint32_t> a(S * m), b(S * m);
    std::vector<uint8_t> minus(S * m, 0);
    for (size_t j = 0; j < S * m; j++) {
      a[j] = pairs[j % m].first;
      b[j] = pairs[j % m].second;
      minus[j] = j >= m;
    }
    check(mc_qgram_common(ctx_, a.data(), b.data(), S == 2 ? minus.data() : nullptr, S * m, q, cnt.data()), "mc_qgram_common");
  }
  for (size_t i = 0; i < m; i++) {
    const uint64_t la = ds_.lengths[pairs[i].first], lb = ds_.lengths[pairs[i].second];
    out[i] = qscreen::below(cnt[i], la, lb, cfg_.cutoff, q) && (S == 1 || qscreen::below(cnt[m + i], la, lb, cfg_.cutoff, q));
  }
}

namespace {
struct HdrKey {
  uint64_t k0, k1;
  uint32_t len, id;
};
HdrKey hdr_key(const Dataset &ds, uint32_t id) {
  const std::string_view h = ds.headers[id];
  unsigned char b[16] = {0};
  memcpy(b, h.data(), h.size() < 16 ? h.size() : 16);
  uint64_t w0 = 0, w1 = 0;
  for (int i = 0; i < 8; i++) {
    w0 = (w0 << 8) | b[i];
    w1 = (w1 << 8) | b[8 + i];
  }
  return HdrKey{w0, w1, (uint32_t)std::min<size_t>(h.size(), 0xffffffffu), id};
}
int hdr_cmp(const Dataset &ds, const HdrKey &x, const HdrKey &y) {
  if (x.k0 != y.k0) return x.k0 < y.k0 ? -1 : 1;
  if (x.k1 != y.k1) return x.k1 < y.k1 ? -1 : 1;
  if (x.len <= 16 && y.len <= 16) return x.len < y.len ? -1 : x.len > y.len ? 1 : 0;
  const int c = ds.headers[x.id].compare(ds.headers[y.id]);
  return c < 0 ? -1 : c > 0 ? 1 : 0;
}
template <typename GetPair>
std::vector<uint32_t> header_set_order(const Dataset &ds, size_t n, GetPair pair_of) {
  struct E {
    HdrKey a, b;
    uint32_t idx;
  };
  std::vector<E> e(n);
  for (size_t i = 0; i < n; i++) {
    const PairId p = pair_of(i);
    e[i] = E{hdr_key(ds, p.first), hdr_key(ds, p.second), (uint32_t)i};
  }
  auto cmp = [&](const E &x, const E &y) {
    const int c = hdr_cmp(ds, x.a, y.a);
    return c != 0 ? c : hdr_cmp(ds, x.b, y.b);
  };
  std::stable_sort(e.begin(), e.end(), [&](const E &x, const E &y) { return cmp(x, y) < 0; });
  std::vector<uint32_t> out;
  out.reserve(n);
  for (size_t i = 0; i < n; i++)
    if (i == 0 || cmp(e[i - 1], e[i]) != 0) out.push_back(e[i].idx);
  return out;
}
}

std::vector<uint32_t> Trainer::length_order(const Dataset &ds, int threads) {
  const size_t N = ds.size();
  std::vector<uint32_t> points(N);
  for (size_t i = 0; i < N; i++) points[i] = (uint32_t)i;
  bool wide = false;
  for (size_t t = 0; t < N; t++) wide |= ds.lengths[t] >> 32 != 0;
  if (wide) {
    std::sort(points.begin(), points.end(),
              [&](uint32_t a, uint32_t b) { return ds.lengths[a] < ds.lengths[b]; });
  } else {
// ... 43 lines not shown
    for (size_t t = 0; t < N; t++) tot += ds_.lengths[t];
    return N > 0 && tot / N > 4096;
  }();
  const int look = [&] {
    const char *e = getenv("MC_NW_LOOKAHEAD");
    const int v = e ? atoi(e) : long_reads ? 1 : 2;
    return v < 1 ? 1 : v > 7 ? 7 : v;
  }();
  const bool spine = [&] {
    const char *e = getenv("MC_NW_SPINE");
    if (e) return atoi(e) != 0;
    return N > 0 && !long_reads;
  }();
  struct Plan {
    std::vector<size_t> pos;
    std::vector<std::array<int, 2>> kid;
  };
  auto tree = [&](size_t p, size_t o, int d, Plan &pl) {
    pl.pos.clear();
    pl.kid.clear();
    if (o == 0) return;
    std::vector<size_t> off;
    pl.pos.push_back(p);
    pl.kid.push_back({-1, -1});
    off.push_back(o);
    std::vector<int> level = {0};
    for (int l = 1; l < d; l++) {
      std::vector<int> next;
      for (int n : level) {
        const size_t oc = off[(size_t)n] / 2;
        if (oc == 0) continue;
        for (int side = 0; side < 2; side++) {
          pl.kid[(size_t)n][(size_t)side] = (int)pl.pos.size();
          next.push_back((int)pl.pos.size());
          pl.pos.push_back(side ? pl.pos[(size_t)n] + off[(size_t)n] : pl.pos[(size_t)n] - off[(size_t)n]);
          pl.kid.push_back({-1, -1});
          off.push_back(oc);
        }
      }
      level.swap(next);
    }
  };
  const int W = cfg_.comm && cfg_.comm->world > 1 ? cfg_.comm->world : 1;
  const size_t per = (P + (size_t)W - 1) / (size_t)W;
  const size_t i0 = std::min(P, per * (size_t)(W > 1 ? cfg_.comm->rank : 0)), i1 = std::min(P, i0 + per);
  const int screen_q = [&] {
    const char *e = getenv("MC_NW_SCREEN");
    if (e && !strcmp(e, "0")) return 0;
    return qscreen::pick_q(cfg_.cutoff);
  }();
  const bool screen_host = [&] {
    const char *e = getenv("MC_NW_SCREEN");
    return !mc_qgram_common || (e && !strcmp(e, "host"));
  }();
  const int spine_gen = (int)std::max<size_t>(1, 2048 / (i1 > i0 ? i1 - i0 : 1));
  const int spine_levels = [&] {
    const char *e = getenv("MC_NW_SPINE_LEVELS");
    const int v = e ? atoi(e) : 0;
    return v > 0 ? v : screen_q ? 64 : spine_gen;
  }();
  const int spine_align = [&] {
    const char *e = getenv("MC_NW_SPINE_ALIGN");
    const int v = e ? atoi(e) : 0;
    return v > 0 ? v : spine_gen;
  }();
  const bool screen_spine = screen_q && !(getenv("MC_NW_SPINE") && atoi(getenv("MC_NW_SPINE")) == 0);
  const int look_deep = [&] {
    const char *e = getenv("MC_NW_LOOKAHEAD");
    return e || long_reads ? look : 5;
  }();
  const bool speculate = !(getenv("MC_NW_SPECULATE") && atoi(getenv("MC_NW_SPECULATE")) == 0);
  bool decisive = false;
  auto left_spine = [&](size_t p, size_t o, Plan &pl) {
    pl.pos.clear();
    pl.kid.clear();
    for (int lv = 0; o > 0 && lv < spine_levels; o /= 2, lv++) {
      if (!pl.pos.empty()) pl.kid.back()[0] = (int)pl.pos.size();
      pl.pos.push_back(p);
      pl.kid.push_back({-1, -1});
      p -= o;
    }
  };
  const uint64_t nw_pairs0 = nw_pairs, nw_cells0 = nw_cells, nw_screened0 = nw_screened;
  {
    Scope s(timer_, "train.sort_keys");
    Scope s3(timer_, "train.sort_keys.pivots");
    if (i1 > i0) check(mc_split_begin(ctx_, indices.data() + i0, (uint32_t)(i1 - i0), points.data(), N), "mc_split_begin");
  }
  std::vector<uint32_t> q_arr, q_ids;
  std::vector<uint64_t> q_pos;
  auto select = [&]() {
    q_ids.resize(q_arr.size());
    if (!q_arr.empty()) {
      std::vector<uint32_t> la(q_arr.size());
      for (size_t q = 0; q < q_arr.size(); q++) la[q] = q_arr[q] - (uint32_t)i0;
      check(mc_split_select(ctx_, q_arr.size(), la.data(), q_pos.data(), q_ids.data()), "mc_split_select");
    }
  };
  std::vector<size_t> offset(P, N / 4), pivot(P, 2 * (N / 4));
  std::vector<char> active(P, 1);
  auto sample_positions = [&](size_t pv, std::vector<size_t> &out) {
    const size_t npts = N;
    double before_inc = (double)pv / to_add_each, after_inc = ((double)(npts - pv)) / to_add_each;
    double bs = 0, as = (double)pv;
    for (int t = 0; t < (int)to_add_each; t++, bs += before_inc) out.push_back((size_t)(int)std::round(bs));
    for (int t = 0; t < (int)to_add_each && std::round(as) < (double)npts; t++, as += after_inc)
      out.push_back((size_t)(int)std::round(as));
  };
  {
    Scope s(timer_, "train.nw_search");
    std::vector<PairId> planned, batch;
    std::vector<size_t> who, first;
    std::vector<char> scr;
    std::vector<int> slot;
    std::vector<Plan> plan(P);
    for (int round = 0;; round++) {
      who.clear();
      for (size_t i = i0; i < i1; i++) {
        if (active[i] && offset[i] == 0) active[i] = 0;
        if (active[i]) who.push_back(i);
      }
      const bool spine_round = round == 0 && (spine || screen_spine);
      {
        Scope s2(timer_, "train.nw_search.resolve");
        first.assign(who.size() + 1, 0);
        q_arr.clear();
        q_pos.clear();
        for (size_t t = 0; t < who.size(); t++) {
          const size_t i = who[t];
          if (spine_round) left_spine(pivot[i], offset[i], plan[i]);
          else tree(pivot[i], offset[i], decisive ? look_deep : look, plan[i]);
          for (size_t n = 0; n < plan[i].pos.size(); n++) {
            q_arr.push_back((uint32_t)i);
            q_pos.push_back(plan[i].pos[n]);
          }
          first[t + 1] = q_arr.size();
        }
        select();
        planned.resize(q_arr.size());
        for (size_t q = 0; q < q_arr.size(); q++) planned[q] = PairId(indices[q_arr[q]], q_ids[q]);
      }
      if (planned.empty()) break;
      {
        Scope s4(timer_, "train.nw_search.screen");
        scr.assign(planned.size(), 0);
        if (screen_q) screen(planned, screen_q, screen_host, scr);
        if (spine_round) {
          size_t roots = 0;
          for (size_t t = 0; t < who.size(); t++) roots += first[t + 1] > first[t] && scr[first[t]];
          decisive = 2 * roots >= who.size() && roots > 0;
        }
        const int round_cap = !spine_round ? 1 << 30 : decisive || !spine ? 0 : spine_align;
        slot.assign(planned.size(), -1);
        batch.clear();
        std::vector<char> need;
        for (size_t t = 0; t < who.size(); t++) {
          const Plan &pl = plan[who[t]];
          const size_t f = first[t];
          need.assign(pl.pos.size(), 0);
          need[0] = 1;
          int aligned = 0;
          for (size_t n = 0; n < pl.pos.size(); n++) {
            if (!need[n]) continue;
            if (scr[f + n]) {
              nw_screened++;
              if (pl.kid[n][0] >= 0) need[(size_t)pl.kid[n][0]] = 1;
              continue;
            }
            if (aligned >= round_cap) continue;
            aligned++;
            slot[f + n] = (int)batch.size();
            batch.push_back(planned[f + n]);
            for (int side = decisive && speculate ? 1 : 0; side < 2; side++)
              if (pl.kid[n][(size_t)side] >= 0) need[(size_t)pl.kid[n][(size_t)side]] = 1;
          }
        }
      }
      std::vector<double> al;
      if (!batch.empty()) {
        Scope s3(timer_, "train.nw_search.align");
        nw_batch(batch, al);
      }
      for (size_t t = 0; t < who.size(); t++) {
        const size_t i = who[t], f = first[t];
        for (int n = 0; n >= 0 && active[i];) {
          const bool below = scr[f + (size_t)n];
          if (!below && slot[f + (size_t)n] < 0) break;
          const double algn = below ? 0.0 : al[(size_t)slot[f + (size_t)n]];
          if (below || algn < cfg_.cutoff) {
            pivot[i] -= offset[i];
            n = plan[i].kid[(size_t)n][0];
          } else if (algn > cfg_.cutoff) {
            pivot[i] += offset[i];
            n = plan[i].kid[(size_t)n][1];
          } else {
            active[i] = 0;
            break;
          }
          offset[i] /= 2;
          if (offset[i] == 0) break;
        }
      }
    }
  }
  int aerr = 0;
  std::vector<std::vector<PairId>> bufs(P);
  {
    Scope sb(timer_, "train.sample");
    q_arr.clear();
    q_pos.clear();
    std::vector<size_t> sp;
    for (size_t i = i0; i < i1; i++) {
      sp.clear();
      sample_positions(pivot[i], sp);
      for (size_t x : sp) {
        q_arr.push_back((uint32_t)i);
        q_pos.push_back(x);
      }
    }
    select();
    for (size_t q = 0; q < q_arr.size(); q++) {
      const uint32_t p = indices[q_arr[q]], x = q_ids[q];
      bufs[q_arr[q]].push_back(hdr_less(p, x) ? PairId(p, x) : PairId(x, p));
    }
    if (i1 > i0) check(mc_split_end(ctx_), "mc_split_end");
    const size_t cap = per * (2 * to_add_each), H = 4;
    std::vector<uint64_t> mine(H + per + cap, 0), all;
    mine[0] = nw_pairs - nw_pairs0;
    mine[1] = nw_cells - nw_cells0;
    mine[3] = nw_screened - nw_screened0;
    size_t np = 0;
    for (size_t i = i0; i < i1; i++) {
      mine[H + (i - i0)] = pivot[i];
      for (const PairId &pr : bufs[i]) mine[H + per + np++] = ((uint64_t)pr.first << 32) | pr.second;
    }
    mine[2] = np;
    if (gather(mine, all)) {
      nw_pairs = nw_pairs0;
      nw_cells = nw_cells0;
      nw_screened = nw_screened0;
      for (int r = 0; r < W; r++) {
        const uint64_t *b = all.data() + (size_t)r * mine.size();
        const size_t r0 = std::min(P, per * (size_t)r), r1 = std::min(P, r0 + per);
        nw_pairs += b[0];
        nw_cells += b[1];
        nw_screened += b[3];
        for (size_t i = r0; i < r1; i++) {
          pivot[i] = b[H + (i - r0)];
          if (r != cfg_.comm->rank) bufs[i].clear();
        }
        if (r == cfg_.comm->rank) continue;
        for (uint64_t q = 0; q < b[2] && r1 > r0; q++)
          bufs[r0].push_back(PairId((uint32_t)(b[H + per + q] >> 32), (uint32_t)b[H + per + q]));
      }
    }
  }
  Scope sp(timer_, "train.sample.pair_set");
  for (size_t i = 0; i < P; i++) {
    double before_inc = (double)pivot[i] / to_add_each;
    double after_inc = ((double)(N - pivot[i])) / to_add_each;
    if (before_inc < 1) aerr = 1;
    else if (after_inc < 1) aerr = -1;
    pairs.insert(pairs.end(), bufs[i].begin(), bufs[i].end());
  }
  {
    const std::vector<uint32_t> ord = header_set_order(ds_, pairs.size(), [&](size_t i) { return pairs[i]; });
    std::vector<PairId> set(ord.size());
    for (size_t i = 0; i < ord.size(); i++) set[i] = pairs[ord[i]];
    pairs.swap(set);
  }
  if (aerr < 0) fprintf(stderr, "Warning: Alignment may be too small for sampling\n");
  else if (aerr > 0) fprintf(stderr, "Warning: Alignment may be too large for sampling\n");
  return pairs;
}

void Trainer::get_labels(const std::vector<PairId> &vec, std::vector<Labeled> &bp, std::vector<Labeled> &bn) {
  std::vector<double> al;
  {
    Scope s(timer_, "train.nw_labels");
    const int W = cfg_.comm && cfg_.comm->world > 1 ? cfg_.comm->world : 1;
    if (W == 1) {
      nw_batch(vec, al);
    } else {
      const size_t m = vec.size(), per = (m + (size_t)W - 1) / (size_t)W;
      const size_t j0 = std::min(m, per * (size_t)cfg_.comm->rank), j1 = std::min(m, j0 + per);
      const uint64_t p0 = nw_pairs, c0 = nw_cells;
      std::vector<double> part;
      nw_batch(std::vector<PairId>(vec.begin() + j0, vec.begin() + j1), part);
      std::vector<uint64_t> mine(2 + per, 0), all;
      mine[0] = nw_pairs - p0;
      mine[1] = nw_cells - c0;
      for (size_t j = j0; j < j1; j++) memcpy(&mine[2 + (j - j0)], &part[j - j0], 8);
      gather(mine, all);
      nw_pairs = p0;
      nw_cells = c0;
      al.assign(m, 0.0);
      for (int r = 0; r < W; r++) {
        const uint64_t *b = all.data() + (size_t)r * mine.size();
        const size_t r0 = std::min(m, per * (size_t)r), r1 = std::min(m, r0 + per);
        nw_pairs += b[0];
        nw_cells += b[1];
        for (size_t j = r0; j < r1; j++) memcpy(&al[j], &b[2 + (j - r0)], 8);
      }
    }
  }
  Scope sl(timer_, "train.label_sets");
  std::vector<Labeled> buf_pos, buf_neg;
  for (size_t i = 0; i < vec.size(); i++) {
    if (al[i] >= cfg_.cutoff) buf_pos.push_back({vec[i], al[i]});
    else buf_neg.push_back({vec[i], al[i]});
  }
  for (std::vector<Labeled> *v : {&buf_pos, &buf_neg}) {
    const std::vector<uint32_t> ord = header_set_order(ds_, v->size(), [&](size_t i) { return (*v)[i].first; });
    std::vector<Labeled> set(ord.size());
    for (size_t i = 0; i < ord.size(); i++) set[i] = (*v)[ord[i]];
    v->swap(set);
  }
  if (cfg_.verbose) printf("positive=%zu negative=%zu\n", buf_pos.size(), buf_neg.size());
  if (buf_pos.empty() || buf_neg.empty()) {
    std::string m = "Identity value does not match sampled data: ";
    m += buf_pos.empty() ? "Too many sequences below identity" : "Too many sequences above identity";
    printf("%s\n", m.c_str());
    throw ExitZero(m);
  }
  size_t m_size = std::min(buf_pos.size(), buf_neg.size());
  std::vector<Labeled> &vpos = buf_pos, &vneg = buf_neg;
  bp = resize_vec(vpos, m_size, cfg_.cutoff, 1, 5);
  bn = resize_vec(vneg, m_size, 0.4, cfg_.cutoff, 5);
  if (cfg_.verbose) printf("positive=%zu negative=%zu\n", bp.size(), bn.size());
}

Matrix Trainer::feat_matrix(const std::vector<PairId> &pos, const std::vector<PairId> &neg, int ncols,
                            Matrix &labels) {
  const size_t n = pos.size() + neg.size();
  Matrix fm((int)n, ncols);
  labels = Matrix((int)n, 1);
  std::vector<uint32_t> a(n), b(n);
  for (size_t i = 0; i < n; i++) {
    const PairId &p = i < pos.size() ? pos[i] : neg[i - pos.size()];
    a[i] = p.first;
    b[i] = p.second;
  }
  const size_t ns = feat.lookup.size();
  std::vector<double> raw(n * ns);
  if (n) check(mc_pair_features(ctx_, a.data(), b.data(), n, feat.lookup.data(), (int)ns, raw.data()), "mc_pair_features");
  for (size_t i = 0; i < n; i++) {
    double *cache = &raw[i * ns];
    feat.normalize_cache(cache);
    fm.set((int)i, 0, 1);
    for (int col = 1; col < ncols; col++) fm.set((int)i, col, feat.combo(col - 1, cache));
    labels.set((int)i, 0, i < pos.size() ? 1 : -1);
  }
  return fm;
}

void Trainer::train(double acc_cutoff) {
  std::pair<std::vector<PairId>, std::vector<PairId>> training, testing;
  if (cfg_.k != 0) {
    if (cfg_.verbose) printf("Splitting data\n");
    split_pairs = split();
    get_labels(split_pairs, label_pos, label_neg);
    auto pos = bin_data(label_pos, cfg_.cutoff, 1);
    training.first = pos.first;
    testing.first = pos.second;
    auto neg = bin_data(label_neg, 0, cfg_.cutoff);
    training.second = neg.first;
    testing.second = neg.second;
    if (cfg_.verbose)
      printf("training positive: %zu\ntraining negative: %zu\ntesting positive: %zu\ntesting negative: %zu\n",
             training.first.size(), training.second.size(), testing.first.size(), testing.second.size());
    if (testing.first.empty() || testing.second.empty()) throw Error("not enough points to sample", 1);
  }
  if (cfg_.k == 0) {
    feat.add_feature(MC_FEAT_ALIGN, MC_COMBO_SELF);
    feat.normalize_with({}, 0);
    feat.finalize();
    weights = {-1 * cfg_.cutoff, 1};
    return;
  }
  Scope s(timer_, "train.glm");
  const std::vector<std::pair<uint16_t, int>> bit_feats = {
      {MC_FEAT_INTERSECTION | MC_FEAT_LD, MC_COMBO_SELF},
      {MC_FEAT_MANHATTAN | MC_FEAT_LD, MC_COMBO_SQUARED},
      {MC_FEAT_PEARSON, MC_COMBO_SELF},
      {MC_FEAT_KULCZYNSKI2 | MC_FEAT_LD, MC_COMBO_SQUARED}};
// ... 58 lines not shown
```

meshclust_amd/csrc/host/trainer.hpp:

```cpp
#pragma once
#include <cstddef>
#include <cstdint>
#include <utility>
#include <vector>

#include "common.hpp"
#include "fasta.hpp"
#include "feature.hpp"
#include "glm.hpp"

namespace mc {

using PairId = std::pair<uint32_t, uint32_t>;

struct TrainerConfig {
  size_t n_points = 3000;
  size_t max_pts_from_one = 20;
  double cutoff = 0.90;
  int k = 4;
  int threads = 1;
  bool verbose = true;
  const ShardComm *comm = nullptr;
  std::vector<uint32_t> length_order;
  bool both_strands = false;
};

class Trainer {
 public:
  Trainer(const Dataset &ds, mc_ctx *ctx, const TrainerConfig &cfg, PhaseTimer &timer)
      : ds_(ds), ctx_(ctx), cfg_(cfg), timer_(timer) {}
  void train(double acc_cutoff = 97.5);
  static std::vector<uint32_t> length_order(const Dataset &ds, int threads);
  mc_classifier classifier() const { return feat.to_classifier(weights); }
  void nw_batch(const std::vector<PairId> &pairs, std::vector<double> &ident);

  FeatureSet feat;
  std::vector<double> weights;
  std::vector<PairId> split_pairs;
  std::vector<std::pair<PairId, double>> label_pos, label_neg;
  uint64_t nw_pairs = 0, nw_cells = 0;
  uint64_t nw_screened = 0;

 private:
  std::vector<PairId> split();
  void get_labels(const std::vector<PairId> &vec, std::vector<std::pair<PairId, double>> &bp,
                  std::vector<std::pair<PairId, double>> &bn);
  Matrix feat_matrix(const std::vector<PairId> &pos, const std::vector<PairId> &neg, int ncols,
                     Matrix &labels);
  bool gather(const std::vector<uint64_t> &mine, std::vector<uint64_t> &all) const;
  bool hdr_less(uint32_t a, uint32_t b) const;
  void screen(const std::vector<PairId> &pairs, int q, bool host, std::vector<char> &out);

  const Dataset &ds_;
  mc_ctx *ctx_;
  TrainerConfig cfg_;
  PhaseTimer &timer_;
};

}
```

Measured before the change: 2.886 million.

## Add banded NW identity kernel with certification and fallback for trainer alignment

Adds a new diagonal-banded Needleman-Wunsch identity kernel (nwdiag) using DPP lane shuffles. Band width comes from the identity cutoff, and the kernel certifies when the banded result is exact, falling back to full NW for uncertified pairs. The trainer's nw_search and nw_labels phases use it by default, and banded and full groups can run concurrently on a side stream. The aim is to cut the DP cells computed per pair, at the cost of extra host bookkeeping, key sorting and gathering, and fallback work when certification fails.

```diff
diff --git a/include/meshclust_amd.h b/include/meshclust_amd.h
--- a/include/meshclust_amd.h
+++ b/include/meshclust_amd.h
@@ -152,6 +152,13 @@
                     int32_t *w , int32_t *score );
 int mc_nw_band_profile(mc_ctx *ctx, double *out , int reset);
 
+#define MC_BAND_REPORT 0
+#define MC_BAND_FALL_THROUGH 1
+int mc_nw_identity_band(mc_ctx *ctx, const uint32_t *a, const uint32_t *b, const uint8_t *a_minus, uint64_t m,
+                        const int32_t *w , int mode, double *ident, int32_t *len, int32_t *ids, int32_t *score,
+                        uint8_t *certified);
+int mc_nw_identity_band_profile(mc_ctx *ctx, double *out , int reset);
+
 #define MC_PILEUP_CH 8
 int mc_nw_pileup_strands(mc_ctx *ctx, const uint32_t *a, const uint32_t *b, const uint8_t *a_minus, uint64_t m,
                          const uint32_t *targets, uint32_t nt, uint64_t *row_off ,
diff --git a/meshclust_amd/__init__.py b/meshclust_amd/__init__.py
--- a/meshclust_amd/__init__.py
+++ b/meshclust_amd/__init__.py
@@ -92,7 +92,8 @@
                      "mc_comm_stats", "mc_comm_destroy", "mc_sync", "mc_assign", "mc_assign_strands",
                      "mc_revcomp_rows", "mc_assign_top", "mc_revcomp_sequences", "mc_nw_identity_strands",
                      "mc_nw_align_strands", "mc_nw_align_profile", "mc_nw_pileup_strands", "mc_nw_pileup_profile",
-                     "mc_kmer_max_strands", "mc_kmer_build_strands", "mc_orient_pairs", "mc_qgram_common"):
+                     "mc_kmer_max_strands", "mc_kmer_build_strands", "mc_orient_pairs", "mc_qgram_common",
+                     "mc_nw_identity_band", "mc_nw_identity_band_profile"):
             getattr(lib, name).restype = C.c_int
         lib.mc_comm_create.argtypes = [C.c_int, C.c_int, C.c_int, C.c_char_p, C.POINTER(C.c_void_p)]
         lib.mc_comm_allgather.argtypes = [C.c_void_p, C.c_void_p, C.c_uint64, C.c_void_p]
@@ -109,6 +110,9 @@
         lib.mc_nw_identity_strands.argtypes = [C.c_void_p, C.c_void_p, C.c_void_p, C.c_void_p, C.c_uint64, C.c_void_p,
                                                C.c_void_p, C.c_void_p]
         lib.mc_qgram_common.argtypes = [C.c_void_p, C.c_void_p, C.c_void_p, C.c_void_p, C.c_uint64, C.c_int, C.c_void_p]
+        lib.mc_nw_identity_band.argtypes = [C.c_void_p, C.c_void_p, C.c_void_p, C.c_void_p, C.c_uint64, C.c_void_p, C.c_int,
+                                            C.c_void_p, C.c_void_p, C.c_void_p, C.c_void_p, C.c_void_p]
+        lib.mc_nw_identity_band_profile.argtypes = [C.c_void_p, C.c_void_p, C.c_int]
         lib.mc_nw_align_strands.argtypes = [C.c_void_p, C.c_void_p, C.c_void_p, C.c_void_p, C.c_uint64, C.c_void_p,
                                             C.c_uint64, C.c_void_p, C.c_void_p, C.c_void_p, C.c_void_p]
         lib.mc_nw_align_profile.argtypes = [C.c_void_p, C.c_void_p, C.c_int]
@@ -574,6 +578,26 @@
         out = np.zeros(len(a), np.uint32)
         self._ck(self.lib.mc_qgram_common(self.ctx, _p(a), _p(b), _p(am), C.c_uint64(len(a)), int(q), _p(out)), "mc_qgram_common")
         return out
+
+    def nw_identity_band(self, a, b, w, fall_through=False, a_minus=None):
+        a = np.ascontiguousarray(a, np.uint32)
+        b = np.ascontiguousarray(b, np.uint32)
+        w = np.ascontiguousarray(w, np.int32)
+        am = None if a_minus is None else np.ascontiguousarray(a_minus, np.uint8)
+        assert len(a) == len(b) == len(w) and (am is None or len(am) == len(a))
+        ident = np.zeros(len(a))
+        ln = np.zeros(len(a), np.int32)
+        ids = np.zeros(len(a), np.int32)
+        score = np.zeros(len(a), np.int32)
+        cert = np.zeros(len(a), np.uint8)
+        self._ck(self.lib.mc_nw_identity_band(self.ctx, _p(a), _p(b), _p(am), C.c_uint64(len(a)), _p(w), 1 if fall_through else 0,
+                                              _p(ident), _p(ln), _p(ids), _p(score), _p(cert)), "mc_nw_identity_band")
+        return ident, ln, ids, score, cert
+
+    def nw_identity_band_profile(self, reset=False):
+        out = np.zeros(5)
+        self._ck(self.lib.mc_nw_identity_band_profile(self.ctx, _p(out), 1 if reset else 0), "mc_nw_identity_band_profile")
+        return dict(zip(("banded", "full", "uncertified", "launches", "swept"), (float(v) for v in out)))
 
     def nw_align_strands(self, a, b, a_minus=None, cigar=True):
         a = np.ascontiguousarray(a, np.uint32)
diff --git a/meshclust_amd/csrc/gpu/abi.hip b/meshclust_amd/csrc/gpu/abi.hip
--- a/meshclust_amd/csrc/gpu/abi.hip
+++ b/meshclust_amd/csrc/gpu/abi.hip
@@ -253,7 +253,7 @@
                  &c->alive, &c->members, &c->member_keys, &c->partials, &c->scan_dev, &c->flags_out, &c->s_a, &c->s_b,
                  &c->s_c, &c->s_d, &c->s_e, &c->s_f, &c->s_g, &c->s_h, &c->s_i, &c->s_j, &c->s_k, &c->hs, &c->mag_s, &c->sumsq_s, &c->len_s, &c->ticket,
                  &c->msum, &c->ident_s, &c->al_a, &c->al_b, &c->al_out, &c->al_id, &c->ord_ids, &c->acc_out, &c->sp_words, &c->sp_keys,
-                 &c->sp_scr, &c->sp_nodes, &c->sp_nn, &c->sp_q, &c->sp_err, &c->u_off, &c->u_mem, &c->nw_items, &c->nw_gran, &c->rc_seq, &c->tr_choice, &c->tr_bnd, &c->tr_ops, &c->tr_pairs, &c->tr_res, &c->tr_idx, &c->tr_dst,
+                 &c->sp_scr, &c->sp_nodes, &c->sp_nn, &c->sp_q, &c->sp_err, &c->u_off, &c->u_mem, &c->nw_items, &c->nw_gran, &c->nd_idx, &c->nd_off, &c->nd_w, &c->nd_bnd, &c->nd_cert, &c->rc_seq, &c->tr_choice, &c->tr_bnd, &c->tr_ops, &c->tr_pairs, &c->tr_res, &c->tr_idx, &c->tr_dst,
                  &c->tr_out, &c->tr_err, &c->bs_pairs, &c->bs_bnd, &c->bs_score, &c->pu_table, &c->pu_diff, &c->pu_rows, &c->pu_toff, &c->pu_roff, &c->qual, &c->pu_wtable, &c->pu_qoff, &c->msa_width, &c->msa_col, &c->msa_words, &c->msa_bw, &c->msa_rec, &c->msa_out, &c->msa_cnt, &c->msa_wcnt, &c->msa_cdiff, &c->msa_crec, &c->msa_ctgt, &c->msa_scol, &c->msa_sres, &c->msa_stgt, &c->msa_srec, &c->msa_sout, &c->msa_sq, &c->msa_xrec, &c->msa_xout, &c->hist_fwd, &c->or_runs})
     release(*b);
   if (c->h_scan) (void)hipHostFree(c->h_scan);
@@ -263,6 +263,9 @@
   for (auto e : c->ev_pool) (void)hipEventDestroy(e);
   (void)hipEventDestroy(c->ev0);
   (void)hipEventDestroy(c->ev1);
+  if (c->band_stream) (void)hipStreamDestroy(c->band_stream);
+  if (c->band_fork) (void)hipEventDestroy(c->band_fork);
+  if (c->band_join) (void)hipEventDestroy(c->band_join);
   (void)hipStreamDestroy(c->stream);
   delete c;
   return MC_OK;
@@ -1235,6 +1238,12 @@
     }
     MCG_CHECK(hipExtStreamCreateWithCUMask(&s, (uint32_t)mask.size(), mask.data()));
   }
+  if (c->band_stream) (void)hipStreamDestroy(c->band_stream);
+  if (c->band_fork) (void)hipEventDestroy(c->band_fork);
+  if (c->band_join) (void)hipEventDestroy(c->band_join);
+  c->band_stream = nullptr;
+  c->band_fork = c->band_join = nullptr;
+  c->band_side_open = false;
   (void)hipStreamDestroy(c->stream);
   c->stream = s;
   c->part_slot = slot;
diff --git a/meshclust_amd/csrc/gpu/abi_align.hip b/meshclust_amd/csrc/gpu/abi_align.hip
--- a/meshclust_amd/csrc/gpu/abi_align.hip
+++ b/meshclust_amd/csrc/gpu/abi_align.hip
@@ -6,6 +6,7 @@
 #include <vector>
 
 #include "../host/band.hpp"
+#include "../host/bandid.hpp"
 #include "../host/pairbatch.hpp"
 #include "abi_util.hpp"
 #include "mcgpu.hpp"
@@ -969,6 +970,116 @@
   return MC_OK;
 }
 
+int mc_nw_identity_band(mc_ctx *c, const uint32_t *a, const uint32_t *b, const uint8_t *a_minus, uint64_t m, const int32_t *w,
+                        int mode, double *ident, int32_t *len, int32_t *ids, int32_t *score, uint8_t *certified) {
+  if (!c || !c->codes.p) return MC_ERR_STATE;
+  if (m == 0) return MC_OK;
+  if (!w || (mode != MC_BAND_REPORT && mode != MC_BAND_FALL_THROUGH)) return MC_ERR_ARG;
+  MCG_CHECK(hipSetDevice(c->device));
+  TRY(check_ids(c, a, m));
+  TRY(check_ids(c, b, m));
+  mc::PairBatcher pb(c->h_seq_off.data(), c->n, a, b, a_minus, m, batch_caps("MC_IDENT_BATCH", MC_IDENT_BATCH_PAIRS, false));
+  std::vector<uint32_t> ai, bi, out;
+  std::vector<uint64_t> h_off, a_off2, la[4], lb[4];
+  std::vector<int32_t> gw[4];
+  std::vector<uint8_t> grp, h_cert;
+  while (pb.next()) {
+    const uint64_t i0 = pb.i0, mb = pb.i1 - pb.i0, nm = pb.nminus;
+    ai.resize(mb);
+    bi.resize(mb);
+    out.resize(mb);
+    grp.resize(mb);
+    uint64_t cnt[4] = {0, 0, 0, 0}, at[4];
+    for (uint64_t i = i0; i < pb.i1; i++) {
+      const bool band = mc::diag_takes((int64_t)pb.length(a[i]), (int64_t)pb.length(b[i]), w[i]);
+      grp[i - i0] = (uint8_t)((pb.minus(i) ? 0 : 2) + (band ? 1 : 0));
+      cnt[grp[i - i0]]++;
+    }
+    at[0] = 0;
+    for (int g = 1; g < 4; g++) at[g] = at[g - 1] + cnt[g - 1];
+    const uint64_t base[4] = {at[0], at[1], at[2], at[3]};
+    for (int g = 0; g < 4; g++) {
+      la[g].clear();
+      lb[g].clear();
+      gw[g].clear();
+    }
+    for (uint64_t i = i0; i < pb.i1; i++) {
+      const int g = grp[i - i0];
+      const uint64_t k = at[g]++;
+      ai[k] = g < 2 ? 2 * pb.slot(a[i]) : a[i];
+      bi[k] = b[i];
+      out[k] = (uint32_t)(i - i0);
+      la[g].push_back(pb.length(a[i]));
+      lb[g].push_back(pb.length(b[i]));
+      gw[g].push_back(w[i]);
+    }
+    if (nm) {
+      TRY(revseq_batch(c, pb.uniq.data(), (uint32_t)pb.uniq.size(), h_off));
+      a_off2.resize(2 * pb.uniq.size());
+      for (size_t r = 0; r < pb.uniq.size(); r++) {
+        a_off2[2 * r] = h_off[r];
+        a_off2[2 * r + 1] = h_off[r] + pb.length(pb.uniq[r]);
+      }
+      TRY(upload(c, c->s_j, a_off2.data(), a_off2.size(), c->stream));
+    }
+    TRY(upload(c, c->s_d, ai.data(), mb, c->stream));
+    TRY(upload(c, c->s_e, bi.data(), mb, c->stream));
+    TRY(upload(c, c->s_g, out.data(), mb, c->stream));
+    TRY(ensure(c->s_f, mb * 20 + 64));
+    TRY(ensure(c->nd_cert, mb + 64));
+    double *d_id = (double *)c->s_f.p;
+    int32_t *d_len = (int32_t *)(d_id + mb), *d_ids = d_len + mb, *d_score = d_ids + mb;
+    uint8_t *d_cert = (uint8_t *)c->nd_cert.p;
+    MCG_CHECK(hipMemsetAsync(d_cert, 1, mb, c->stream));
+    const uint32_t *d_ai = (const uint32_t *)c->s_d.p, *d_bi = (const uint32_t *)c->s_e.p, *d_out = (const uint32_t *)c->s_g.p;
+    static const bool overlap_on = [] {
+      const char *e = getenv("MC_NW_BAND_OVERLAP");
+      return !(e && atoi(e) == 0);
+    }();
+    const bool side = overlap_on && c->part_share <= 1 && cnt[0] + cnt[2] > 0 && cnt[1] + cnt[3] > 0;
+    const int first[4] = {0, 2, 1, 3}, side_first[4] = {1, 3, 0, 2};
+    for (int gi = 0; gi < 4; gi++) {
+      const int g = side ? side_first[gi] : first[gi];
+      if (cnt[g] == 0) continue;
+      const uint8_t *A = g < 2 ? (const uint8_t *)c->rc_seq.p : (const uint8_t *)c->codes.p;
+      const uint64_t *aoff = g < 2 ? (const uint64_t *)c->s_j.p : (const uint64_t *)c->seq_off.p;
+      if (g & 1) {
+        TRY(launch_nwdiag(c, A, aoff, d_ai + base[g], (uint8_t *)c->codes.p, (uint64_t *)c->seq_off.p, d_bi + base[g], cnt[g], la[g],
+                          lb[g], gw[g], mode == MC_BAND_FALL_THROUGH, d_id, d_len, d_ids, d_score, d_cert, d_out + base[g], side));
+        c->bandid_stat[0] += (double)cnt[g];
+        c->bandid_stat[3] += 1;
+        for (uint64_t k = 0; k < cnt[g]; k++)
+          c->bandid_stat[4] += (double)mc::diag_swept(la[g][k], lb[g][k], mc::diag_lane_k((int64_t)la[g][k], (int64_t)lb[g][k], gw[g][k]));
+      } else {
+        TRY(launch_nw(c, A, aoff, d_ai + base[g], (uint8_t *)c->codes.p, (uint64_t *)c->seq_off.p, d_bi + base[g], cnt[g], la[g], lb[g],
+                      d_id, d_len, d_ids, d_score, d_out + base[g]));
+        c->bandid_stat[1] += (double)cnt[g];
+      }
+    }
+    if (side) {
+      timed_begin(c);
+      TRY(nwdiag_join(c));
+      timed_end(c, F_NW);
+    }
+    h_cert.resize(mb);
+    TRY(download_parts(c, {{ident ? ident + i0 : nullptr, d_id, mb * 8}, {len ? len + i0 : nullptr, d_len, mb * 4},
+                           {ids ? ids + i0 : nullptr, d_ids, mb * 4}, {score ? score + i0 : nullptr, d_score, mb * 4},
+                           {h_cert.data(), d_cert, mb}}, c->stream));
+    for (uint64_t k = 0; k < mb; k++) c->bandid_stat[2] += h_cert[k] ? 0 : 1;
+    if (certified) memcpy(certified + i0, h_cert.data(), mb);
+  }
+  flush_timers(c);
+  return MC_OK;
+}
+
+int mc_nw_identity_band_profile(mc_ctx *c, double *out, int reset) {
+  if (!c || !out) return MC_ERR_ARG;
+  for (int k = 0; k < 5; k++) out[k] = c->bandid_stat[k];
+  if (reset)
+    for (double &v : c->bandid_stat) v = 0;
+  return MC_OK;
+}
+
 int mc_nw_align_strands(mc_ctx *c, const uint32_t *a, const uint32_t *b, const uint8_t *a_minus, uint64_t m,
                         uint32_t *cigar, uint64_t cap, uint64_t *cig_off, int32_t *score, int32_t *len, int32_t *ids) {
   if (!c || !c->codes.p) return MC_ERR_STATE;
diff --git a/meshclust_amd/csrc/gpu/mcgpu.hpp b/meshclust_amd/csrc/gpu/mcgpu.hpp
--- a/meshclust_amd/csrc/gpu/mcgpu.hpp
+++ b/meshclust_amd/csrc/gpu/mcgpu.hpp
@@ -168,6 +168,11 @@
   int part_slot = 0, part_share = 1, part_cus = 0;
   mcg::Buf s_a, s_b, s_c, s_d, s_e, s_f, s_g, s_h, s_i, s_j, s_k;
   mcg::Buf nw_items, nw_gran;
+  double bandid_stat[5] = {0, 0, 0, 0, 0};
+  hipStream_t band_stream = nullptr;
+  hipEvent_t band_fork = nullptr, band_join = nullptr;
+  bool band_side_open = false;
+  mcg::Buf nd_idx, nd_off, nd_w, nd_bnd, nd_cert;
   mcg::Buf rc_seq;
   mcg::Buf tr_choice, tr_bnd, tr_ops, tr_pairs, tr_res, tr_idx, tr_dst, tr_out, tr_err;
   double tr_choice_bytes = 0;
@@ -250,6 +255,11 @@
               const uint64_t *d_boff, const uint32_t *d_bi, uint64_t m, const std::vector<uint64_t> &h_alen,
               const std::vector<uint64_t> &h_blen, double *d_ident, int32_t *d_len, int32_t *d_ids,
               int32_t *d_score, const uint32_t *d_out = nullptr);
+int launch_nwdiag(mc_ctx *c, const uint8_t *d_A, const uint64_t *d_aoff, const uint32_t *d_ai, const uint8_t *d_B,
+                  const uint64_t *d_boff, const uint32_t *d_bi, uint64_t m, const std::vector<uint64_t> &h_alen,
+                  const std::vector<uint64_t> &h_blen, const std::vector<int32_t> &h_w, bool fall_through, double *d_ident,
+                  int32_t *d_len, int32_t *d_ids, int32_t *d_score, uint8_t *d_cert, const uint32_t *d_out, bool side = false);
+int nwdiag_join(mc_ctx *c);
 int launch_revseq(mc_ctx *c, const uint32_t *d_ids, uint32_t u, const uint64_t *d_out_off, uint64_t out_bytes,
                   uint8_t *d_out);
 
diff --git a/meshclust_amd/csrc/gpu/nwdiag.hip b/meshclust_amd/csrc/gpu/nwdiag.hip
--- /dev/null
+++ b/meshclust_amd/csrc/gpu/nwdiag.hip
@@ -0,0 +1,477 @@
+#include <algorithm>
+
+#include "../host/bandid.hpp"
+#include "mcgpu.hpp"
+
+namespace mcg {
+
+namespace {
+
+constexpr int GO = 2, GE = 1, MATCH = 1, MISMATCH = -1;
+constexpr int OPEN_T = GO + GE - 1, EXT_T = 1 - GE, MATCH_T = MATCH + 2, MISMATCH_T = MISMATCH + 2;
+constexpr int MOFF = OPEN_T;
+constexpr int SENT = mc::BAND_SENTINEL;
+constexpr uint32_t LEN1 = 1u << 16;
+constexpr int FULL_R = 8;
+
+__device__ __forceinline__ int from_below(int v) { return __builtin_amdgcn_mov_dpp(v, 0x138, 0xf, 0xf, false); }
+__device__ __forceinline__ int from_above(int v) { return __builtin_amdgcn_mov_dpp(v, 0x130, 0xf, 0xf, false); }
+
+struct DiagArgs {
+  const uint8_t *A;
+  const uint64_t *aoff;
+  const uint32_t *ai;
+  const uint8_t *Bq;
+  const uint64_t *boff;
+  const uint32_t *bi;
+  const uint32_t *pidx;
+  uint32_t npairs;
+  const int32_t *w;
+  int fall_through;
+  int *bnd;
+  const uint64_t *bnd_off;
+  double *ident;
+  int32_t *len;
+  int32_t *ids;
+  int32_t *score;
+  uint8_t *cert;
+  const uint32_t *out;
+};
+
+__device__ __forceinline__ int neg_inf(int la, int lb) {
+  const int shorter = la < lb ? la : lb;
+  const int lenDiff = la > lb ? la - lb : lb - la;
+  int maxDiff = 0;
+  if (lenDiff >= 1) maxDiff += -GO - lenDiff * GE;
+  return maxDiff + MISMATCH * shorter - 1;
+}
+
+template <int K>
+__device__ __forceinline__ void diag_run(const uint8_t *__restrict__ a, const int la, const uint8_t *__restrict__ b, const int lb,
+                                         const int dlo, const int NINF, const int lane, int &fin_score, uint32_t &fin_pay) {
+  constexpr int H = K / 2;
+  const int d0 = dlo + K * lane;
+  int M[K], X[K], Y[K];
+  uint32_t MP[K], XP[K], YP[K];
+#pragma unroll
+  for (int k = 0; k < K; k++) {
+    const int d = d0 + k;
+    MP[k] = XP[k] = YP[k] = 0;
+    if (d > lb || d < -la) {
+      M[k] = X[k] = Y[k] = SENT;
+    } else if (d == 0) {
+      M[k] = -MOFF;
+      X[k] = NINF;
+      Y[k] = -GO;
+    } else if (d > 0) {
+      M[k] = NINF + d - MOFF;
+      X[k] = NINF + d;
+      Y[k] = -GO - d * GE + d;
+    } else {
+      M[k] = NINF - d - MOFF;
+      Y[k] = NINF - d;
+      X[k] = -GO + d * GE - d;
+    }
+  }
+  const int t0 = 2 - (dlo & 1), tend = la + lb;
+  const int iA0 = (t0 - d0) / 2, jA0 = (t0 + d0) / 2;
+  uint32_t awin = 0, bwin = 0;
+#pragma unroll
+  for (int m = 0; m < H; m++) {
+    const int i = iA0 - m, j = jA0 + m;
+    const uint32_t ca = (i >= 1 && i <= la) ? a[i - 1] : 0u, cb = (j >= 1 && j <= lb) ? b[j - 1] : 0u;
+    awin |= ca << (8 * m);
+    bwin |= cb << (8 * m);
+  }
+  const int fa = (t0 - dlo) / 2, fb = (t0 + dlo + 63 * K) / 2 + H - 1;
+  auto base_at = [&](const uint8_t *s, int len, int idx) -> int { return (idx >= 0 && idx < len) ? (int)s[idx] : 0; };
+  int acur = 0, anext = base_at(a, la, fa + lane), bcur = 0, bnext = base_at(b, lb, fb + lane);
+  const bool lane0 = lane == 0, lane63 = lane == 63;
+
+  auto cell = [&](int k, int loM, int loY, uint32_t loMP, uint32_t loYP, int hiM, int hiX, uint32_t hiMP, uint32_t hiXP, bool hit,
+                  bool commit) {
+    const bool yFromM = loM >= loY + EXT_T;
+    const int Yn = yFromM ? loM : loY + EXT_T;
+    const uint32_t YPn = yFromM ? loMP : loYP;
+    const bool xy = X[k] >= Y[k];
+    const int mxy = xy ? X[k] : Y[k];
+    const uint32_t pxy = xy ? XP[k] : YP[k];
+    const int m2 = mxy - MOFF;
+    const bool fromM = M[k] >= m2;
+    const int best = fromM ? M[k] : m2;
+    const uint32_t bestP = fromM ? MP[k] : pxy;
+    const int Mn = best + (hit ? MATCH_T : MISMATCH_T);
+    const uint32_t MPn = bestP + LEN1 + (hit ? 1u : 0u);
+    const bool xFromM = hiM >= hiX + EXT_T;
+    const int Xn = xFromM ? hiM : hiX + EXT_T;
+    const uint32_t XPn = xFromM ? hiMP : hiXP;
+    if (commit) {
+      M[k] = Mn;
+      X[k] = Xn;
+      Y[k] = Yn;
+      MP[k] = MPn;
+      XP[k] = XPn;
+      YP[k] = YPn;
+    }
+  };
+  auto inside = [&](int i, int j) { return (unsigned)(i - 1) < (unsigned)la && (unsigned)(j - 1) < (unsigned)lb; };
+
+  auto pair = [&](int n, auto gen_tag) {
+    constexpr bool GEN = decltype(gen_tag)::value;
+    if ((n & 63) == 0) {
+      acur = anext;
+      bcur = bnext;
+      anext = base_at(a, la, fa + n + 64 + lane);
+      bnext = base_at(b, lb, fb + n + 64 + lane);
+    }
+    const uint32_t a_in = (uint32_t)__builtin_amdgcn_readlane(acur, n & 63);
+    const uint32_t b_in = (uint32_t)__builtin_amdgcn_readlane(bcur, n & 63);
+    const int iA = iA0 + n, jA = jA0 + n;
+    {
+      int nM = from_below(M[K - 1]), nY = from_below(Y[K - 1]);
+      const uint32_t nMP = (uint32_t)from_below((int)MP[K - 1]), nYP = (uint32_t)from_below((int)YP[K - 1]);
+      nM = lane0 ? SENT : nM;
+      nY = lane0 ? SENT : nY;
+      const uint32_t x = awin ^ bwin;
+#pragma unroll
+      for (int m = 0; m < H; m++) {
+        const int k = 2 * m;
+        const bool hit = ((x >> (8 * m)) & 0xffu) == 0;
+        const bool ok = !GEN || inside(iA - m, jA + m);
+        const int kl = k > 0 ? k - 1 : 0;
+        if (k == 0) cell(k, nM, nY, nMP, nYP, M[k + 1], X[k + 1], MP[k + 1], XP[k + 1], hit, ok);
+        else cell(k, M[kl], Y[kl], MP[kl], YP[kl], M[k + 1], X[k + 1], MP[k + 1], XP[k + 1], hit, ok);
+      }
+    }
+    {
+      uint32_t in = (uint32_t)from_above((int)(bwin & 0xffu));
+      in = lane63 ? b_in : in;
+      bwin = (bwin >> 8) | (in << (8 * (H - 1)));
+    }
+    {
+      int nM = from_above(M[0]), nX = from_above(X[0]);
+      const uint32_t nMP = (uint32_t)from_above((int)MP[0]), nXP = (uint32_t)from_above((int)XP[0]);
+      nM = lane63 ? SENT : nM;
+      nX = lane63 ? SENT : nX;
+      const uint32_t x = awin ^ bwin;
+#pragma unroll
+      for (int m = 0; m < H; m++) {
+        const int k = 2 * m + 1;
+        const bool hit = ((x >> (8 * m)) & 0xffu) == 0;
+        const bool ok = !GEN || inside(iA - m, jA + 1 + m);
+        const int kh = k + 1 < K ? k + 1 : k;
+        if (k == K - 1) cell(k, M[k - 1], Y[k - 1], MP[k - 1], YP[k - 1], nM, nX, nMP, nXP, hit, ok);
+        else cell(k, M[k - 1], Y[k - 1], MP[k - 1], YP[k - 1], M[kh], X[kh], MP[kh], XP[kh], hit, ok);
+      }
+    }
+    {
+      uint32_t in = (uint32_t)from_below((int)((awin >> (8 * (H - 1))) & 0xffu));
+      in = lane0 ? a_in : in;
+      awin = (awin << 8) | in;
+    }
+  };
+  const int dtop = dlo + 64 * K - 1;
+  const int tlo = max(-dlo, dtop) + 2, thi = min(2 * la + dlo, 2 * lb - dtop) - 1;
+  const int npair = (tend - t0) / 2 + 1;
+  const int n_lo = min(npair, max(0, (tlo - t0 + 1) / 2));
+  const int n_hi = min(npair, max(n_lo, thi >= t0 ? (thi - t0) / 2 + 1 : 0));
+  int n = 0;
+  for (; n < n_lo; n++) pair(n, std::true_type{});
+  for (; n < n_hi; n++) pair(n, std::false_type{});
+  for (; n < npair; n++) pair(n, std::true_type{});
+  const int kk = (lb - la) - dlo;
+  if (lane == kk / K) {
+    const int kf = kk % K;
+    int mM = 0, mX = 0, mY = 0;
+    uint32_t pM = 0, pX = 0, pY = 0;
+#pragma unroll
+    for (int k = 0; k < K; k++)
+      if (k == kf) {
+        mM = M[k] + MOFF;
+        mX = X[k];
+        mY = Y[k];
+        pM = MP[k];
+        pX = XP[k];
+        pY = YP[k];
+      }
+    int sc = mM > mX ? mM : mX;
+    sc = sc > mY ? sc : mY;
+    fin_score = sc - (la + lb);
+    fin_pay = sc == mM ? pM : (sc == mX ? pX : pY);
+  }
+}
+
+template <int R>
+__device__ __forceinline__ void full_run(const uint8_t *a, const int la, const uint8_t *b, const int lb, const int NINF, int *bnd,
+                                      const int lane, int &fin_score, uint32_t &fin_pay) {
+  constexpr int ROWS = 64 * R;
+  const int nblk = (la + ROWS - 1) / ROWS;
+  for (int blk = 0; blk < nblk; blk++) {
+    const int itop = blk * ROWS + lane * R + 1;
+    uint8_t ac[R];
+    int M[R], X[R], Y[R];
+    uint32_t MP[R], XP[R], YP[R];
+#pragma unroll
+    for (int r = 0; r < R; r++) {
+      const int i = itop + r;
+      ac[r] = i <= la ? a[i - 1] : (uint8_t)0xFF;
+      M[r] = NINF + i - MOFF;
+      Y[r] = NINF + i;
+      X[r] = -GO - i * GE + i;
+      MP[r] = XP[r] = YP[r] = 0;
+    }
+    int dM, dX, dY;
+    uint32_t dMP = 0, dXP = 0, dYP = 0;
+    {
+      const int i = itop - 1;
+      if (i == 0) {
+        dM = -MOFF;
+        dX = NINF;
+        dY = -GO;
+      } else {
+        dM = NINF + i - MOFF;
+        dX = -GO - i * GE + i;
+        dY = NINF + i;
+      }
+    }
+    int oM = NINF, oX = NINF, oY = NINF, ob = 0;
+    uint32_t oMP = 0, oXP = 0, oYP = 0;
+    const int steps = lb + 63;
+    int bcur = 0, bnext = lane < lb ? b[lane] : 0;
+    for (int t = 0; t < steps; t++) {
+      const int j = t - lane + 1;
+      if ((t & 63) == 0) {
+        bcur = bnext;
+        const int nx = t + 64 + lane;
+        bnext = nx < lb ? b[nx] : 0;
+      }
+      const int b0 = __builtin_amdgcn_readlane(bcur, t & 63);
+      int uM = from_below(oM), uX = from_below(oX), uY = from_below(oY);
+      uint32_t uMP = (uint32_t)from_below((int)oMP), uXP = (uint32_t)from_below((int)oXP), uYP = (uint32_t)from_below((int)oYP);
+      int bc = from_below(ob);
+      const bool in = j >= 1 && j <= lb;
+      if (lane == 0) {
+        bc = in ? b0 : 0;
+        if (in) {
+          if (blk == 0) {
+            uM = NINF + j - MOFF;
+            uX = NINF + j;
+            uY = -GO - j * GE + j;
+            uMP = uXP = uYP = 0;
+          } else {
+            const int *sb = bnd + 6 * j;
+            uM = sb[0];
+            uX = sb[1];
+            uY = sb[2];
+            uMP = (uint32_t)sb[3];
+            uXP = (uint32_t)sb[4];
+            uYP = (uint32_t)sb[5];
+          }
+        }
+      }
+      if (in) {
+        int aM = uM, aX = uX;
+        uint32_t aMP = uMP, aXP = uXP;
+        int gM = dM, gX = dX, gY = dY;
+        uint32_t gMP = dMP, gXP = dXP, gYP = dYP;
+#pragma unroll
+        for (int r = 0; r < R; r++) {
+          const int pM = M[r], pX = X[r], pY = Y[r];
+          const uint32_t pMP = MP[r], pXP = XP[r], pYP = YP[r];
+          const int yb = pM, yc = pY + EXT_T;
+          const bool yFromM = yb >= yc;
+          Y[r] = yFromM ? yb : yc;
+          YP[r] = yFromM ? pMP : pYP;
+          const bool hit = ac[r] == (uint8_t)bc;
+          const int sc = hit ? MATCH_T : MISMATCH_T;
+          const bool xy = gX >= gY;
+          const int mxy = xy ? gX : gY;
+          const uint32_t pxy = xy ? gXP : gYP;
+          const int m2 = mxy - MOFF;
+          const bool fromM = gM >= m2;
+          const int best = fromM ? gM : m2;
+          const uint32_t bestP = fromM ? gMP : pxy;
+          M[r] = best + sc;
+          MP[r] = bestP + LEN1 + (hit ? 1u : 0u);
+          const int xb = aM, xc = aX + EXT_T;
+          const bool xFromM = xb >= xc;
+          X[r] = xFromM ? xb : xc;
+          XP[r] = xFromM ? aMP : aXP;
+          aM = M[r];
+          aX = X[r];
+          aMP = MP[r];
+          aXP = XP[r];
+          gM = pM;
+          gX = pX;
+          gY = pY;
+          gMP = pMP;
+          gXP = pXP;
+          gYP = pYP;
+        }
+        dM = uM;
+        dX = uX;
+        dY = uY;
+        dMP = uMP;
+        dXP = uXP;
+        dYP = uYP;
+        oM = M[R - 1];
+        oX = X[R - 1];
+        oY = Y[R - 1];
+        oMP = MP[R - 1];
+        oXP = XP[R - 1];
+        oYP = YP[R - 1];
+        if (lane == 63 && blk + 1 < nblk) {
+          int *sb = bnd + 6 * j;
+          sb[0] = oM;
+          sb[1] = oX;
+          sb[2] = oY;
+          sb[3] = (int)oMP;
+          sb[4] = (int)oXP;
+          sb[5] = (int)oYP;
+        }
+      }
+      ob = bc;
+    }
+    const int fl = la - blk * ROWS - 1;
+    if (fl >= 0 && fl < ROWS && lane == fl / R) {
+      const int r = fl % R;
+      int mM = 0, mX = 0, mY = 0;
+      uint32_t pM = 0, pX = 0, pY = 0;
+#pragma unroll
+      for (int rr = 0; rr < R; rr++)
+        if (rr == r) {
+          mM = M[rr] + MOFF;
+          mX = X[rr];
+          mY = Y[rr];
+          pM = MP[rr];
+          pX = XP[rr];
+          pY = YP[rr];
+        }
+      int sc = mM > mX ? mM : mX;
+      sc = sc > mY ? sc : mY;
+      fin_score = sc - (la + lb);
+      fin_pay = sc == mM ? pM : (sc == mX ? pX : pY);
+    }
+    __threadfence_block();
+    __syncthreads();
+  }
+}
+
+__global__ __launch_bounds__(64) void nw_diag_kernel(DiagArgs q) {
+  const uint32_t slot = blockIdx.x;
+  if (slot >= q.npairs) return;
+  const uint32_t p = q.pidx[slot];
+  const uint8_t *a = q.A + q.aoff[q.ai[p]];
+  const int la = (int)(q.aoff[q.ai[p] + 1] - q.aoff[q.ai[p]]);
+  const uint8_t *b = q.Bq + q.boff[q.bi[p]];
+  const int lb = (int)(q.boff[q.bi[p] + 1] - q.boff[q.bi[p]]);
+  const int w = q.w[p];
+  const int lane = (int)threadIdx.x;
+  const int NINF = neg_inf(la, lb);
+  const int diff = la > lb ? la - lb : lb - la, shorter = la < lb ? la : lb;
+  const int dlo = (lb < la ? lb - la : 0) - w;
+  const int K = 2 * ((2 * w + diff + 1 + 127) / 128);
+  int fs = 0;
+  uint32_t fp = 0;
+  switch (K) {
+    case 2: diag_run<2>(a, la, b, lb, dlo, NINF, lane, fs, fp); break;
+    case 4: diag_run<4>(a, la, b, lb, dlo, NINF, lane, fs, fp); break;
+    case 6: diag_run<6>(a, la, b, lb, dlo, NINF, lane, fs, fp); break;
+    default: diag_run<8>(a, la, b, lb, dlo, NINF, lane, fs, fp); break;
+  }
+  const uint32_t o = q.out ? q.out[p] : p;
+  const bool owner = lane == ((lb - la) - dlo) / K;
+  const bool certified = fs > NINF + shorter && fs > shorter - diff - 3 * (w + 1) - 4;
+  bool redo = false;
+  if (owner) {
+    if (certified || !q.fall_through) {
+      const int L = certified ? la + lb - (int)(fp >> 16) : 0, I = certified ? (int)(fp & 0xffffu) : 0;
+      q.ident[o] = certified ? (double)I / (double)L : 0.0;
+      if (q.len) q.len[o] = L;
+      if (q.ids) q.ids[o] = I;
+      if (q.score) q.score[o] = certified ? fs : 0;
+      if (q.cert) q.cert[o] = certified ? 1 : 0;
+    } else {
+      redo = true;
+    }
+  }
+  if (__ballot(redo) == 0) return;
+  full_run<FULL_R>(a, la, b, lb, NINF, q.bnd + q.bnd_off[slot], lane, fs, fp);
+  if (lane == ((la - 1) % (64 * FULL_R)) / FULL_R) {
+    const int L = la + lb - (int)(fp >> 16), I = (int)(fp & 0xffffu);
+    q.ident[o] = (double)I / (double)L;
+    if (q.len) q.len[o] = L;
+    if (q.ids) q.ids[o] = I;
+    if (q.score) q.score[o] = fs;
+    if (q.cert) q.cert[o] = 0;
+  }
+}
+
+}
+
+int launch_nwdiag(mc_ctx *c, const uint8_t *d_A, const uint64_t *d_aoff, const uint32_t *d_ai, const uint8_t *d_B,
+                  const uint64_t *d_boff, const uint32_t *d_bi, uint64_t m, const std::vector<uint64_t> &alen,
+                  const std::vector<uint64_t> &blen, const std::vector<int32_t> &h_w, bool fall_through, double *d_ident,
+                  int32_t *d_len, int32_t *d_ids, int32_t *d_score, uint8_t *d_cert, const uint32_t *d_out, bool side) {
+  if (m == 0) return MC_OK;
+  std::vector<uint64_t> cost(m);
+  for (uint64_t i = 0; i < m; i++) {
+    const int k = mc::diag_lane_k((int64_t)alen[i], (int64_t)blen[i], h_w[i]);
+    if (k == 0 || alen[i] + blen[i] >= 65535) {
+      set_error("launch_nwdiag: a pair the diagonal kernel does not take");
+      return MC_ERR_ARG;
+    }
+    cost[i] = mc::diag_swept(alen[i], blen[i], k);
+  }
+  std::vector<uint32_t> order(m);
+  for (uint64_t i = 0; i < m; i++) order[i] = (uint32_t)i;
+  std::stable_sort(order.begin(), order.end(), [&](uint32_t x, uint32_t y) { return cost[x] > cost[y]; });
+  std::vector<uint64_t> boff(m, 0);
+  uint64_t scratch = 0;
+  if (fall_through)
+    for (uint64_t s = 0; s < m; s++) {
+      const uint64_t i = order[s];
+      boff[s] = scratch;
+      if (alen[i] > 64ull * FULL_R) scratch += 6 * (blen[i] + 2);
+    }
+  if (ensure(c->nd_idx, m * 4 + 16) || ensure(c->nd_off, m * 8 + 16) || ensure(c->nd_w, m * 4 + 16) ||
+      ensure(c->nd_bnd, std::max<uint64_t>(scratch, 1) * 4))
+    return MC_ERR_OOM;
+  if (side) {
+    if (!c->band_stream) {
+      MCG_CHECK(hipStreamCreateWithFlags(&c->band_stream, hipStreamNonBlocking));
+      MCG_CHECK(hipEventCreateWithFlags(&c->band_fork, hipEventDisableTiming));
+      MCG_CHECK(hipEventCreateWithFlags(&c->band_join, hipEventDisableTiming));
+    }
+    if (int rc = nwdiag_join(c)) return rc;
+  } else {
+    timed_begin(c);
+  }
+  if (int rc = stage_h2d(c, c->nd_idx.p, order.data(), m * 4)) return rc;
+  if (int rc = stage_h2d(c, c->nd_off.p, boff.data(), m * 8)) return rc;
+  if (int rc = stage_h2d(c, c->nd_w.p, h_w.data(), m * 4)) return rc;
+  DiagArgs q{d_A, d_aoff, d_ai, d_B, d_boff, d_bi, (const uint32_t *)c->nd_idx.p, (uint32_t)m, (const int32_t *)c->nd_w.p,
+             fall_through ? 1 : 0, (int *)c->nd_bnd.p, (const uint64_t *)c->nd_off.p, d_ident, d_len, d_ids, d_score, d_cert, d_out};
+  if (side) {
+    MCG_CHECK(hipEventRecord(c->band_fork, c->stream));
+    MCG_CHECK(hipStreamWaitEvent(c->band_stream, c->band_fork, 0));
+    nw_diag_kernel<<<(uint32_t)m, 64, 0, c->band_stream>>>(q);
+    MCG_CHECK(hipGetLastError());
+    MCG_CHECK(hipEventRecord(c->band_join, c->band_stream));
+    c->band_side_open = true;
+    return MC_OK;
+  }
+  nw_diag_kernel<<<(uint32_t)m, 64, 0, c->stream>>>(q);
+  MCG_CHECK(hipGetLastError());
+  timed_end(c, F_NW);
+  return MC_OK;
+}
+
+int nwdiag_join(mc_ctx *c) {
+  if (!c->band_side_open) return MC_OK;
+  MCG_CHECK(hipStreamWaitEvent(c->stream, c->band_join, 0));
+  c->band_side_open = false;
+  return MC_OK;
+}
+
+}
diff --git a/meshclust_amd/csrc/host/bandid.hpp b/meshclust_amd/csrc/host/bandid.hpp
--- /dev/null
+++ b/meshclust_amd/csrc/host/bandid.hpp
@@ -0,0 +1,44 @@
+#pragma once
+#include <algorithm>
+#include <cstdint>
+
+#include "band.hpp"
+
+namespace mc {
+
+constexpr int DIAG_KMAX = 8;
+constexpr double BANDID_MARGIN = 1e-9;
+
+inline int64_t diag_count(int64_t la, int64_t lb, int64_t w) { return 2 * w + (la > lb ? la - lb : lb - la) + 1; }
+
+inline int diag_lane_k(int64_t la, int64_t lb, int64_t w) {
+  if (la <= 0 || lb <= 0 || w < 0) return 0;
+  const int64_t nd = diag_count(la, lb, w);
+  const int64_t k = 2 * ((nd + 127) / 128);
+  return k <= DIAG_KMAX ? (int)k : 0;
+}
+
+inline bool diag_takes(int64_t la, int64_t lb, int64_t w) { return la + lb < 65535 && diag_lane_k(la, lb, w) != 0; }
+
+inline uint64_t diag_swept(uint64_t la, uint64_t lb, int k) { return 32ull * (uint64_t)k * (la + lb); }
+
+inline int32_t band_w_lemma(int64_t la, int64_t lb, double cutoff) {
+  const double c = cutoff - BANDID_MARGIN;
+  if (!(c > 0.75) || la <= 0 || lb <= 0) return -1;
+  const int64_t m = std::max(la, lb);
+  const int64_t T = (int64_t)((4.0 * c - 3.0) * (double)m);
+  const int64_t diff = la > lb ? la - lb : lb - la;
+  const int64_t q = std::min(la, lb) - diff - 4 - T;
+  const int64_t w = q < 0 ? 0 : q / 3;
+  return w >= (1 << 27) ? -1 : (int32_t)w;
+}
+
+inline int32_t band_w_cutoff(int64_t la, int64_t lb, double cutoff) {
+  const int32_t w = band_w_lemma(la, lb, cutoff);
+  if (w < 0) return -1;
+  const int k = diag_lane_k(la, lb, w);
+  if (k == 0 || la + lb >= 65535 || 20 * diag_swept((uint64_t)la, (uint64_t)lb, k) > 13 * (uint64_t)la * (uint64_t)lb) return -1;
+  return w;
+}
+
+}
diff --git a/meshclust_amd/csrc/host/cluster.hpp b/meshclust_amd/csrc/host/cluster.hpp
--- a/meshclust_amd/csrc/host/cluster.hpp
+++ b/meshclust_amd/csrc/host/cluster.hpp
@@ -38,6 +38,7 @@
   uint64_t update_evals_run = 0;
   uint64_t nw_pairs = 0, nw_cells = 0;
   uint64_t nw_screened = 0;
+  uint64_t nw_banded = 0, nw_band_uncertified = 0, nw_band_fallback = 0;
   uint64_t align_nw_pairs = 0, align_nw_cells = 0;
   std::string accum_path;
   std::string update_path;
diff --git a/meshclust_amd/csrc/host/common.hpp b/meshclust_amd/csrc/host/common.hpp
--- a/meshclust_amd/csrc/host/common.hpp
+++ b/meshclust_amd/csrc/host/common.hpp
@@ -17,6 +17,8 @@
 int mc_nw_identity_strands(mc_ctx *, const uint32_t *, const uint32_t *, const uint8_t *, uint64_t, double *, int32_t *,
                            int32_t *) __attribute__((weak));
 int mc_qgram_common(mc_ctx *, const uint32_t *, const uint32_t *, const uint8_t *, uint64_t, int, uint32_t *) __attribute__((weak));
+int mc_nw_identity_band(mc_ctx *, const uint32_t *, const uint32_t *, const uint8_t *, uint64_t, const int32_t *, int, double *,
+                        int32_t *, int32_t *, int32_t *, uint8_t *) __attribute__((weak));
 }
 
 namespace mc {
diff --git a/meshclust_amd/csrc/host/runner.cpp b/meshclust_amd/csrc/host/runner.cpp
--- a/meshclust_amd/csrc/host/runner.cpp
+++ b/meshclust_amd/csrc/host/runner.cpp
@@ -365,6 +365,9 @@
   rr.stats.nw_pairs = tr.nw_pairs;
   rr.stats.nw_cells = tr.nw_cells;
   rr.stats.nw_screened = tr.nw_screened;
+  rr.stats.nw_banded = tr.nw_banded;
+  rr.stats.nw_band_uncertified = tr.nw_band_uncertified;
+  rr.stats.nw_band_fallback = tr.nw_band_fallback;
   if (opt.both_strands) {
     Scope s(rr.timer, "orient");
     std::vector<uint32_t> a, b;
@@ -412,6 +415,9 @@
   if (!rr.stats.update_path.empty()) o += ", \"update_path\": \"" + rr.stats.update_path + "\"";
   o += ", \"update_iters_fixed\": " + std::to_string(rr.stats.update_iters_fixed);
   o += ", \"update_evals_run\": " + std::to_string(rr.stats.update_evals_run);
+  o += ", \"nw_banded\": " + std::to_string(rr.stats.nw_banded);
+  o += ", \"nw_band_uncertified\": " + std::to_string(rr.stats.nw_band_uncertified);
+  o += ", \"nw_band_fallback\": " + std::to_string(rr.stats.nw_band_fallback);
   o += ", \"phases_ms\": {";
   for (size_t i = 0; i < rr.timer.order.size(); i++) {
     snprintf(b, sizeof b, "%s\"%s\": %.3f", i ? ", " : "", rr.timer.order[i].c_str(), rr.timer.ms.at(rr.timer.order[i]));
diff --git a/meshclust_amd/csrc/host/trainer.cpp b/meshclust_amd/csrc/host/trainer.cpp
--- a/meshclust_amd/csrc/host/trainer.cpp
+++ b/meshclust_amd/csrc/host/trainer.cpp
@@ -1,6 +1,7 @@
 #include "trainer.hpp"
 
 #include "lazysort.hpp"
+#include "bandid.hpp"
 #include "qscreen.hpp"
 
 #include <algorithm>
@@ -105,6 +106,53 @@
   check(mc_nw_identity_strands(ctx_, a.data(), b.data(), minus.data(), 2 * m, both.data(), nullptr, nullptr),
         "mc_nw_identity_strands");
   for (size_t i = 0; i < m; i++) ident[i] = both[m + i] > both[i] ? both[m + i] : both[i];
+}
+
+bool Trainer::band_on() const {
+  static const bool env_on = [] {
+    const char *e = getenv("MC_NW_BAND");
+    return !(e && !strcmp(e, "0"));
+  }();
+  return env_on && mc_nw_identity_band && cfg_.cutoff - BANDID_MARGIN > 0.75;
+}
+
+void Trainer::nw_batch_band(const std::vector<PairId> &pairs, const std::vector<char> &want, bool fall_through,
+                            std::vector<double> &ident) {
+  const size_t m = pairs.size(), S = cfg_.both_strands ? 2 : 1;
+  ident.assign(m, 0.0);
+  if (m == 0) return;
+  if (S == 2) strands_engine_check();
+  std::vector<uint32_t> a(S * m), b(S * m);
+  std::vector<uint8_t> minus(S * m, 0), cert(S * m, 0);
+  std::vector<int32_t> w(S * m);
+  std::vector<double> val(S * m, 0.0);
+  for (size_t j = 0; j < S * m; j++) {
+    const PairId &p = pairs[j % m];
+    const uint64_t la = ds_.lengths[p.first], lb = ds_.lengths[p.second];
+    a[j] = p.first;
+    b[j] = p.second;
+    minus[j] = j >= m;
+    w[j] = want[j % m] ? band_w_cutoff((int64_t)la, (int64_t)lb, cfg_.cutoff) : -1;
+    nw_pairs++;
+    if (w[j] >= 0) {
+      nw_banded++;
+      nw_cells += diag_swept(la, lb, diag_lane_k((int64_t)la, (int64_t)lb, w[j]));
+    } else {
+      nw_cells += la * lb;
+    }
+  }
+  check(mc_nw_identity_band(ctx_, a.data(), b.data(), S == 2 ? minus.data() : nullptr, S * m, w.data(),
+                            fall_through ? MC_BAND_FALL_THROUGH : MC_BAND_REPORT, val.data(), nullptr, nullptr, nullptr, cert.data()),
+        "mc_nw_identity_band");
+  for (size_t j = 0; j < S * m; j++) {
+    if (cert[j]) continue;
+    nw_band_uncertified++;
+    if (fall_through) {
+      nw_band_fallback++;
+      nw_cells += ds_.lengths[a[j]] * ds_.lengths[b[j]];
+    }
+  }
+  for (size_t i = 0; i < m; i++) ident[i] = S == 2 && val[m + i] > val[i] ? val[m + i] : val[i];
 }
 
 void Trainer::screen(const std::vector<PairId> &pairs, int q, bool host, std::vector<char> &out) {
@@ -314,6 +362,7 @@
     }
   };
   const uint64_t nw_pairs0 = nw_pairs, nw_cells0 = nw_cells, nw_screened0 = nw_screened;
+  const uint64_t nw_band0[3] = {nw_banded, nw_band_uncertified, nw_band_fallback};
   {
     Scope s(timer_, "train.sort_keys");
     Scope s3(timer_, "train.sort_keys.pivots");
@@ -411,7 +460,8 @@
       std::vector<double> al;
       if (!batch.empty()) {
         Scope s3(timer_, "train.nw_search.align");
-        nw_batch(batch, al);
+        if (band_on()) nw_batch_band(batch, std::vector<char>(batch.size(), 1), false, al);
+        else nw_batch(batch, al);
       }
       for (size_t t = 0; t < who.size(); t++) {
         const size_t i = who[t], f = first[t];
@@ -437,6 +487,7 @@
   }
   int aerr = 0;
   std::vector<std::vector<PairId>> bufs(P);
+  before_keys_.clear();
   {
     Scope sb(timer_, "train.sample");
     q_arr.clear();
@@ -454,13 +505,19 @@
     for (size_t q = 0; q < q_arr.size(); q++) {
       const uint32_t p = indices[q_arr[q]], x = q_ids[q];
       bufs[q_arr[q]].push_back(hdr_less(p, x) ? PairId(p, x) : PairId(x, p));
+      if (q_pos[q] < pivot[q_arr[q]]) before_keys_.push_back(((uint64_t)bufs[q_arr[q]].back().first << 32) | bufs[q_arr[q]].back().second);
     }
     if (i1 > i0) check(mc_split_end(ctx_), "mc_split_end");
-    const size_t cap = per * (2 * to_add_each), H = 4;
-    std::vector<uint64_t> mine(H + per + cap, 0), all;
+    const size_t cap = per * (2 * to_add_each), H = 8;
+    std::vector<uint64_t> mine(H + per + 2 * cap, 0), all;
     mine[0] = nw_pairs - nw_pairs0;
     mine[1] = nw_cells - nw_cells0;
     mine[3] = nw_screened - nw_screened0;
+    mine[4] = nw_banded - nw_band0[0];
+    mine[5] = nw_band_uncertified - nw_band0[1];
+    mine[6] = nw_band_fallback - nw_band0[2];
+    mine[7] = std::min(before_keys_.size(), cap);
+    for (size_t q = 0; q < (size_t)mine[7]; q++) mine[H + per + cap + q] = before_keys_[q];
     size_t np = 0;
     for (size_t i = i0; i < i1; i++) {
       mine[H + (i - i0)] = pivot[i];
@@ -471,12 +528,20 @@
       nw_pairs = nw_pairs0;
       nw_cells = nw_cells0;
       nw_screened = nw_screened0;
+      nw_banded = nw_band0[0];
+      nw_band_uncertified = nw_band0[1];
+      nw_band_fallback = nw_band0[2];
+      before_keys_.clear();
       for (int r = 0; r < W; r++) {
         const uint64_t *b = all.data() + (size_t)r * mine.size();
         const size_t r0 = std::min(P, per * (size_t)r), r1 = std::min(P, r0 + per);
         nw_pairs += b[0];
         nw_cells += b[1];
         nw_screened += b[3];
+        nw_banded += b[4];
+        nw_band_uncertified += b[5];
+        nw_band_fallback += b[6];
+        before_keys_.insert(before_keys_.end(), b + H + per + cap, b + H + per + cap + b[7]);
         for (size_t i = r0; i < r1; i++) {
           pivot[i] = b[H + (i - r0)];
           if (r != cfg_.comm->rank) bufs[i].clear();
@@ -487,6 +552,7 @@
       }
     }
   }
+  std::sort(before_keys_.begin(), before_keys_.end());
   Scope sp(timer_, "train.sample.pair_set");
   for (size_t i = 0; i < P; i++) {
     double before_inc = (double)pivot[i] / to_add_each;
@@ -511,28 +577,46 @@
   {
     Scope s(timer_, "train.nw_labels");
     const int W = cfg_.comm && cfg_.comm->world > 1 ? cfg_.comm->world : 1;
+    const bool band = band_on();
+    auto align = [&](const std::vector<PairId> &v, std::vector<double> &out) {
+      if (!band) return nw_batch(v, out);
+      std::vector<char> want(v.size());
+      for (size_t i = 0; i < v.size(); i++)
+        want[i] = std::binary_search(before_keys_.begin(), before_keys_.end(), ((uint64_t)v[i].first << 32) | v[i].second);
+      nw_batch_band(v, want, true, out);
+    };
     if (W == 1) {
-      nw_batch(vec, al);
+      align(vec, al);
     } else {
       const size_t m = vec.size(), per = (m + (size_t)W - 1) / (size_t)W;
       const size_t j0 = std::min(m, per * (size_t)cfg_.comm->rank), j1 = std::min(m, j0 + per);
-      const uint64_t p0 = nw_pairs, c0 = nw_cells;
+      const uint64_t p0 = nw_pairs, c0 = nw_cells, bd0[3] = {nw_banded, nw_band_uncertified, nw_band_fallback};
       std::vector<double> part;
-      nw_batch(std::vector<PairId>(vec.begin() + j0, vec.begin() + j1), part);
-      std::vector<uint64_t> mine(2 + per, 0), all;
+      align(std::vector<PairId>(vec.begin() + j0, vec.begin() + j1), part);
+      const size_t LH = 5;
+      std::vector<uint64_t> mine(LH + per, 0), all;
       mine[0] = nw_pairs - p0;
       mine[1] = nw_cells - c0;
-      for (size_t j = j0; j < j1; j++) memcpy(&mine[2 + (j - j0)], &part[j - j0], 8);
+      mine[2] = nw_banded - bd0[0];
+      mine[3] = nw_band_uncertified - bd0[1];
+      mine[4] = nw_band_fallback - bd0[2];
+      for (size_t j = j0; j < j1; j++) memcpy(&mine[LH + (j - j0)], &part[j - j0], 8);
       gather(mine, all);
       nw_pairs = p0;
       nw_cells = c0;
+      nw_banded = bd0[0];
+      nw_band_uncertified = bd0[1];
+      nw_band_fallback = bd0[2];
       al.assign(m, 0.0);
       for (int r = 0; r < W; r++) {
         const uint64_t *b = all.data() + (size_t)r * mine.size();
         const size_t r0 = std::min(m, per * (size_t)r), r1 = std::min(m, r0 + per);
         nw_pairs += b[0];
         nw_cells += b[1];
-        for (size_t j = r0; j < r1; j++) memcpy(&al[j], &b[2 + (j - r0)], 8);
+        nw_banded += b[2];
+        nw_band_uncertified += b[3];
+        nw_band_fallback += b[4];
+        for (size_t j = r0; j < r1; j++) memcpy(&al[j], &b[LH + (j - r0)], 8);
       }
     }
   }
diff --git a/meshclust_amd/csrc/host/trainer.hpp b/meshclust_amd/csrc/host/trainer.hpp
--- a/meshclust_amd/csrc/host/trainer.hpp
+++ b/meshclust_amd/csrc/host/trainer.hpp
@@ -40,6 +40,7 @@
   std::vector<std::pair<PairId, double>> label_pos, label_neg;
   uint64_t nw_pairs = 0, nw_cells = 0;
   uint64_t nw_screened = 0;
+  uint64_t nw_banded = 0, nw_band_uncertified = 0, nw_band_fallback = 0;
 
  private:
   std::vector<PairId> split();
@@ -50,6 +51,9 @@
   bool gather(const std::vector<uint64_t> &mine, std::vector<uint64_t> &all) const;
   bool hdr_less(uint32_t a, uint32_t b) const;
   void screen(const std::vector<PairId> &pairs, int q, bool host, std::vector<char> &out);
+  bool band_on() const;
+  void nw_batch_band(const std::vector<PairId> &pairs, const std::vector<char> &want, bool fall_through, std::vector<double> &ident);
+  std::vector<uint64_t> before_keys_;
 
   const Dataset &ds_;
   mc_ctx *ctx_;
```

New measurement: 2.813 million. -2.5%, worse.
